# Kolkir/feature-point-cnn

Measured on AMD Instinct MI355X. Metric: frames/sec (VGA 640x480) SuperPoint fwd+NMS+descriptors, higher is better.
Workload: dtype f32

## Files before the change

feature-point-cnn_amd/_lib.py:

```python
import ctypes
import os
import subprocess

import torch

_DIR = os.path.dirname(os.path.abspath(__file__))
LIB_PATH = os.environ.get("FPC_LIB_PATH") or os.path.join(_DIR, "lib", "libfpc.so")
CSRC = os.path.join(_DIR, "csrc")

SYMBOLS = [
    "fpc_abi_version", "fpc_build_flags", "fpc_strerror", "fpc_last_hip_error", "fpc_default_config", "fpc_create",
    "fpc_destroy", "fpc_load_weights", "fpc_packed_size", "fpc_packed_device_ptr",
    "fpc_export_packed", "fpc_import_packed", "fpc_import_packed_device", "fpc_mark_weights_loaded", "fpc_set_stream", "fpc_upload_stream",
    "fpc_get_stream", "fpc_sync", "fpc_forward", "fpc_detect", "fpc_get_points", "fpc_results",
    "fpc_get_counts", "fpc_get_keypoints", "fpc_set_timing", "fpc_get_timings", "fpc_match", "fpc_first_within",
    "fpc_detect_u8", "fpc_u8_staging", "fpc_homography_adaptation", "fpc_detect_u8_resized",
    "fpc_sample_descriptors", "fpc_plan_hash", "fpc_broadcast_weights", "fpc_read_activation",
    "fpc_pack_layout_revision", "fpc_check_guards", "fpc_stream_report", "fpc_output_range",
    "fpc_match_frames", "fpc_first_within_frames",
    "fpc_default_ransac_params", "fpc_ransac_homography", "fpc_homography_frames",
    "fpc_bank_create", "fpc_bank_destroy", "fpc_bank_get", "fpc_bank_store", "fpc_bank_store_rows", "fpc_bank_clear",
    "fpc_match_bank", "fpc_homography_bank", "fpc_bank_create_ex", "fpc_bank_format",
    "fpc_match_frames_guided", "fpc_match_bank_guided",
    "fpc_cell_order", "fpc_match_frames_guided_cells", "fpc_match_bank_guided_cells",
    "fpc_bank_topk_reserve", "fpc_match_bank_topk", "fpc_homography_bank_topk",
    "fpc_ransac_fundamental", "fpc_fundamental_frames", "fpc_fundamental_bank",
    "fpc_match_frames_guided_epipolar", "fpc_match_bank_guided_epipolar",
    "fpc_match_frames_guided_epipolar_cells", "fpc_match_bank_guided_epipolar_cells",
    "fpc_default_pose_params", "fpc_pose_fundamental", "fpc_pose_frames", "fpc_pose_bank",
    "fpc_default_pnp_params", "fpc_pnp_reserve", "fpc_bank_landmarks_reserve", "fpc_bank_store_landmarks",
    "fpc_bank_landmarks_get", "fpc_ransac_pnp", "fpc_pnp_frames", "fpc_pnp_bank",
]

ABI_VERSION = 4
PACK_LAYOUT_REVISION = 4

PLAN_FLAGS = {
    "no_fused_blocks": 1 << 0, "no_winograd": 1 << 1, "no_winograd_detector": 1 << 2, "no_winograd_layer_in1": 1 << 3,
    "no_xcd_order": 1 << 4, "no_fused_stem_pool": 1 << 5, "split_heads": 1 << 6, "nms_in_line": 1 << 7,
    "no_persistent_grid": 1 << 8, "layer1_tile_8x16": 1 << 9, "winograd_gen1": 1 << 10, "no_latency_tiles": 1 << 11,
    "nms_one_workgroup": 1 << 12, "no_fused_softmax": 1 << 13, "winograd_gen2": 1 << 14, "guard_zones": 1 << 15, "detector_gen1": 1 << 16, "heads_in_line": 1 << 17, "w36_one_wave": 1 << 18, "convt_phases": 1 << 19, "stem_round3": 1 << 20, "conv_round1": 1 << 21,
}


class FpcConfig(ctypes.Structure):
    _fields_ = [("device", ctypes.c_int), ("height", ctypes.c_int), ("width", ctypes.c_int),
                ("max_batch", ctypes.c_int), ("cell", ctypes.c_int), ("nms_dist", ctypes.c_int),
                ("conf_thresh", ctypes.c_float), ("border_remove", ctypes.c_int),
                ("descriptor_enabled", ctypes.c_int), ("max_keypoints", ctypes.c_int),
                ("in_channels", ctypes.c_int), ("dtype", ctypes.c_int), ("arch", ctypes.c_int),
                ("num_streams", ctypes.c_int), ("plan_flags", ctypes.c_uint), ("nms_round_launches", ctypes.c_int),
                ("min_sub_batch", ctypes.c_int)]


class FpcTensor(ctypes.Structure):
    _fields_ = [("name", ctypes.c_char_p), ("data", ctypes.c_void_p), ("ndim", ctypes.c_int),
                ("shape", ctypes.c_int64 * 4)]


class FpcDeviceResults(ctypes.Structure):
    _fields_ = [("count", ctypes.c_void_p), ("n_candidates", ctypes.c_void_p), ("xy", ctypes.c_void_p),
                ("conf", ctypes.c_void_p), ("desc", ctypes.c_void_p), ("capacity", ctypes.c_int),
                ("desc_dim", ctypes.c_int)]


class FpcStreamReport(ctypes.Structure):
    _fields_ = [("n_streams", ctypes.c_int), ("slot", ctypes.c_int * 16), ("queue", ctypes.c_int * 16),
                ("probing", ctypes.c_int), ("hw_queues_found", ctypes.c_int), ("process_probe_rounds", ctypes.c_int),
                ("process_probe_launches", ctypes.c_int), ("process_inconclusive_rounds", ctypes.c_int),
                ("process_probe_ms", ctypes.c_float), ("create_probe_rounds", ctypes.c_int),
                ("create_placement_ms", ctypes.c_float), ("process_registered_streams", ctypes.c_int)]


class FpcRansacParams(ctypes.Structure):
    _fields_ = [("iterations", ctypes.c_int), ("reproj_threshold", ctypes.c_float), ("seed", ctypes.c_uint32),
                ("refits", ctypes.c_int), ("min_inliers", ctypes.c_int)]


class FpcPoseParams(ctypes.Structure):
    _fields_ = [("q_fx", ctypes.c_float), ("q_fy", ctypes.c_float), ("q_cx", ctypes.c_float), ("q_cy", ctypes.c_float),
                ("t_fx", ctypes.c_float), ("t_fy", ctypes.c_float), ("t_cx", ctypes.c_float), ("t_cy", ctypes.c_float),
                ("reproj_threshold", ctypes.c_float), ("min_front", ctypes.c_int)]


class FpcPnpParams(ctypes.Structure):
    _fields_ = [("fx", ctypes.c_float), ("fy", ctypes.c_float), ("cx", ctypes.c_float), ("cy", ctypes.c_float),
                ("iterations", ctypes.c_int), ("reproj_threshold", ctypes.c_float), ("seed", ctypes.c_uint32),
                ("refits", ctypes.c_int), ("min_inliers", ctypes.c_int)]


BANK_MAX_SLOTS = 1024
BANK_TOPK_MAX = 16


# ... 73 lines not shown
    l.fpc_first_within_frames.argtypes = [vp, ci, vp, vp, ctypes.c_float, vp]
    rp = ctypes.POINTER(FpcRansacParams)
    l.fpc_default_ransac_params.argtypes = [rp]
    l.fpc_ransac_homography.argtypes = [vp, ci, vp, vp, vp, ci, rp, vp, vp, vp]
    l.fpc_homography_frames.argtypes = [vp, ci, ci, vp, vp, vp, rp, vp, vp, vp]
    l.fpc_bank_create.argtypes = [vp, ci, ci]
    l.fpc_bank_create_ex.argtypes = [vp, ci, ci, ci]
    l.fpc_bank_format.argtypes = [vp, ctypes.POINTER(ci), ctypes.POINTER(vp)]
    l.fpc_bank_destroy.argtypes = [vp]
    l.fpc_bank_get.argtypes = [vp, ctypes.POINTER(FpcBankView)]
    l.fpc_bank_store.argtypes = [vp, ci, ci]
    l.fpc_bank_store_rows.argtypes = [vp, ci, vp, vp, vp]
    l.fpc_bank_clear.argtypes = [vp, ci]
    l.fpc_match_bank.argtypes = [vp, ci, ci, ctypes.c_float, ctypes.c_float, ci, vp, vp, vp, vp]
    l.fpc_homography_bank.argtypes = [vp, ci, vp, vp, rp, vp, vp, vp]
    l.fpc_ransac_fundamental.argtypes = [vp, ci, vp, vp, vp, ci, rp, vp, vp, vp]
    l.fpc_fundamental_frames.argtypes = [vp, ci, ci, vp, vp, vp, rp, vp, vp, vp]
    l.fpc_fundamental_bank.argtypes = [vp, ci, vp, vp, rp, vp, vp, vp]
    pp = ctypes.POINTER(FpcPoseParams)
    l.fpc_default_pose_params.argtypes = [pp]
    l.fpc_pose_fundamental.argtypes = [vp, ci, vp, vp, vp, ci, vp, pp, vp, vp, vp, vp, vp]
    l.fpc_pose_frames.argtypes = [vp, ci, ci, vp, vp, vp, vp, pp, vp, vp, vp, vp, vp]
    l.fpc_pose_bank.argtypes = [vp, ci, vp, vp, vp, pp, vp, vp, vp, vp, vp]
    np_ = ctypes.POINTER(FpcPnpParams)
    l.fpc_default_pnp_params.argtypes = [np_]
    l.fpc_pnp_reserve.argtypes = [vp, ctypes.POINTER(ctypes.c_size_t)]
    l.fpc_bank_landmarks_reserve.argtypes = [vp, ctypes.POINTER(ctypes.c_size_t)]
    l.fpc_bank_store_landmarks.argtypes = [vp, ci, vp, vp]
    l.fpc_bank_landmarks_get.argtypes = [vp, ctypes.POINTER(vp)]
    l.fpc_ransac_pnp.argtypes = [vp, ci, vp, vp, vp, ci, np_, vp, vp, vp, vp]
    l.fpc_pnp_frames.argtypes = [vp, ci, vp, vp, vp, vp, np_, vp, vp, vp, vp]
    l.fpc_pnp_bank.argtypes = [vp, ci, vp, vp, np_, vp, vp, vp, vp]
    l.fpc_match_frames_guided.argtypes = [vp, ci, ci, vp, vp, vp, vp, ctypes.c_float, ci, ctypes.c_float, ctypes.c_float,
                                          vp, vp]
    l.fpc_match_bank_guided.argtypes = [vp, ci, vp, vp, ctypes.c_float, ci, ctypes.c_float, ctypes.c_float, vp, vp]
    l.fpc_cell_order.argtypes = [vp, vp, vp, ci, ci, vp]
    l.fpc_match_frames_guided_cells.argtypes = [vp, ci, ci, vp, vp, vp, vp, ctypes.c_float, ci, ctypes.c_float,
                                                ctypes.c_float, vp, vp, vp]
    l.fpc_match_bank_guided_cells.argtypes = [vp, ci, vp, vp, ctypes.c_float, ci, ctypes.c_float, ctypes.c_float, vp, vp,
                                              vp]
    l.fpc_match_frames_guided_epipolar.argtypes = list(l.fpc_match_frames_guided.argtypes)
    l.fpc_match_bank_guided_epipolar.argtypes = list(l.fpc_match_bank_guided.argtypes)
    l.fpc_match_frames_guided_epipolar_cells.argtypes = list(l.fpc_match_frames_guided_cells.argtypes)
    l.fpc_match_bank_guided_epipolar_cells.argtypes = list(l.fpc_match_bank_guided_cells.argtypes)
    l.fpc_bank_topk_reserve.argtypes = [vp, ci, ctypes.POINTER(ctypes.c_size_t)]
    l.fpc_match_bank_topk.argtypes = [vp, ci, ci, ci, ctypes.c_float, ctypes.c_float, ci, vp, vp, vp, vp, vp]
    l.fpc_homography_bank_topk.argtypes = [vp, ci, ci, vp, vp, rp, vp, vp, vp, vp, vp]
    l.fpc_sample_descriptors.argtypes = [vp, vp, vp, ci, vp]
    l.fpc_read_activation.argtypes = [vp, ctypes.c_char_p, ci, ci, vp, ctypes.POINTER(ci), ctypes.POINTER(ci), ctypes.POINTER(ci)]
    l.fpc_plan_hash.argtypes = [vp]
    l.fpc_plan_hash.restype = ctypes.c_uint64
    l.fpc_broadcast_weights.argtypes = [vp, vp, ci]
    l.fpc_pack_layout_revision.restype = ci
    l.fpc_check_guards.argtypes = [vp, ctypes.POINTER(ctypes.c_longlong)]
    l.fpc_stream_report.argtypes = [vp, ctypes.POINTER(FpcStreamReport)]
    l.fpc_set_timing.argtypes = [vp, ci]
    l.fpc_get_timings.argtypes = [vp, ci, ctypes.POINTER(ctypes.c_char_p), ctypes.POINTER(ctypes.c_char_p),
                                  ctypes.POINTER(ctypes.c_float), ctypes.POINTER(ctypes.c_double),
                                  ctypes.POINTER(ctypes.c_double), ctypes.POINTER(ctypes.c_double)]
    for s in SYMBOLS:
        getattr(l, s)
    if l.fpc_abi_version() != ABI_VERSION:
        raise ImportError("libfpc.so has ABI version %d, this binding is for %d: rebuild (make -C %s)"
                          % (l.fpc_abi_version(), ABI_VERSION, CSRC))
    if l.fpc_pack_layout_revision() != PACK_LAYOUT_REVISION:
        raise ImportError("libfpc.so packs fragment-layout revision %d, this binding expects %d: rebuild (make -C %s)"
                          % (l.fpc_pack_layout_revision(), PACK_LAYOUT_REVISION, CSRC))
    _lib = l
    return l


def check(code, where):
    if code < 0:
        raise FpcError(code, where)
    return code
```

feature-point-cnn_amd/csrc/fpc_api.hip:

```cpp
#include <hip/hip_runtime.h>

#include <dlfcn.h>

#include <algorithm>
#include <cmath>
#include <cstdio>
#include <cstdlib>
#include <cstring>
#include <memory>
#include <mutex>
#include <chrono>
#include <string>
#include <vector>

#include "../../include/fpc.h"
#include "block_mfma.h"
#include "block_bf16.h"
#include "convt_bf16.h"
#include "block_x3.h"
#include "stem_bf16.h"
#include "wblock_mfma.h"
#include "wblock16_mfma.h"
#include "wblock36_mfma.h"
#include "wblock36p_mfma.h"
// ... 70 lines not shown
FPC_KINDS(X)
#undef X

static const KindInfo g_kinds[K_COUNT] = {
#define X(name, TH, TW, S, EXT, KC, WM, WN, MB, NB)                                                    \
  {#name, "conv_mfma_kernel<" #TH ", " #TW ", " #S ", " #EXT ", " #KC ", " #WM ", " #WN ", " #MB ", " #NB ">", TH, TW, S, EXT, KC, WM, WN, MB, NB, ConvCfg<TH, TW, S, EXT, KC, WM, WN, MB, NB>::LDS_BYTES,   \
   WM * WN * 64, (const void*)conv_mfma_kernel<TH, TW, S, EXT, KC, WM, WN, MB, NB>, launch_##name},
    FPC_KINDS(X)
#undef X
};

#define FPC_LEAN_KINDS(X)                          \
  X(T320_2x2_K64_N128, 3, 20, 1, 2, 64, 1, 4, 2, 1) \
  X(T320_1x1_K64_N128, 3, 20, 1, 1, 64, 1, 4, 2, 1)
struct LeanKindInfo {
  Kind kind;
  const char* symbol;
  int lds_bytes;
  const void* fn;
  void (*launch)(const ConvArgs&, dim3, hipStream_t);
};
#define X(name, TH, TW, S, EXT, KC, WM, WN, MB, NB)                                                              \
  static void launch_lean_##name(const ConvArgs& a, dim3 grid, hipStream_t st) {                                 \
    using C2 = Conv2Cfg<TH, TW, S, EXT, KC, WM, WN, MB, NB>;                                                    \
    hipLaunchKernelGGL((conv2_mfma_kernel<TH, TW, S, EXT, KC, WM, WN, MB, NB>), grid, dim3(WM* WN * 64),         \
                       C2::LDS_BYTES, st, a);                                                                    \
  }
FPC_LEAN_KINDS(X)
#undef X
static const LeanKindInfo g_lean_kinds[] = {
#define X(name, TH, TW, S, EXT, KC, WM, WN, MB, NB)                                                                       \
  {K_##name, "conv2_mfma_kernel<" #TH ", " #TW ", " #S ", " #EXT ", " #KC ", " #WM ", " #WN ", " #MB ", " #NB ">",          \
   Conv2Cfg<TH, TW, S, EXT, KC, WM, WN, MB, NB>::LDS_BYTES, (const void*)conv2_mfma_kernel<TH, TW, S, EXT, KC, WM, WN, MB, NB>, \
   launch_lean_##name},
    FPC_LEAN_KINDS(X)
#undef X
};
static const LeanKindInfo* lean_kind(Kind k) {
  for (const LeanKindInfo& l : g_lean_kinds)
    if (l.kind == k) return &l;
  return nullptr;
}

#define FPC_BLOCK_KINDS(X)                                   \
  X(B816_s1_K64_C64, 8, 16, 1, 64, 4, 1, 1, 2, 64)           \
  X(B1616_s1_K32_C64, 16, 16, 1, 32, 4, 1, 2, 2, 64)         \
  X(B620_s2_K32_C128, 6, 20, 2, 32, 2, 2, 2, 2, 128)         \
  X(B620_s1_K64_C128, 6, 20, 1, 64, 2, 2, 2, 2, 128)         \
  X(B620_s1_K64_C72, 6, 20, 1, 64, 4, 1, 1, 3, 72)           \
  X(B620_s1_K72_C72, 6, 20, 1, 72, 4, 1, 1, 3, 72)           \
  X(B320_s2_K32_C256, 3, 20, 2, 32, 1, 4, 2, 2, 256)         \
  X(B310_s2_K32_C256, 3, 10, 2, 32, 1, 4, 1, 2, 256)         \
  X(B320_s2_K32_C128, 3, 20, 2, 32, 1, 4, 2, 1, 128)         \
  X(B320_s1_K64_C256, 3, 20, 1, 64, 1, 4, 2, 2, 256)

enum BKind {
#define X(name, ...) BK_##name,
  FPC_BLOCK_KINDS(X)
#undef X
      BK_COUNT
};

struct BKindInfo {
  const char* name;
  const char* symbol;
  int TH, TW, S, KC, WM, WN, MB, NB, CMIDP;
  int lds_bytes;
  const void* fn;
  void (*launch)(const BlockArgs&, dim3, hipStream_t);
};

#define X(name, TH, TW, S, KC, WM, WN, MB, NB, CMIDP)                                                     \
  static void launchb_##name(const BlockArgs& a, dim3 grid, hipStream_t st) {                             \
    using BC = BlockCfg<TH, TW, S, KC, WM, WN, MB, NB, CMIDP>;                                            \
    hipLaunchKernelGGL((block_mfma_kernel<TH, TW, S, KC, WM, WN, MB, NB, CMIDP>), grid, dim3(WM* WN * 64), \
                       BC::LDS_BYTES, st, a);                                                             \
  }
FPC_BLOCK_KINDS(X)
#undef X

static const BKindInfo g_bkinds[BK_COUNT] = {
#define X(name, TH, TW, S, KC, WM, WN, MB, NB, CMIDP)                                                      \
  {#name, "block_mfma_kernel<" #TH ", " #TW ", " #S ", " #KC ", " #WM ", " #WN ", " #MB ", " #NB ", " #CMIDP ">", \
   TH, TW, S, KC, WM, WN, MB, NB, CMIDP, BlockCfg<TH, TW, S, KC, WM, WN, MB, NB, CMIDP>::LDS_BYTES,         \
   (const void*)block_mfma_kernel<TH, TW, S, KC, WM, WN, MB, NB, CMIDP>, launchb_##name},
    FPC_BLOCK_KINDS(X)
#undef X
};

#define FPC_WBLOCK_KINDS(X)     \
  X(W816_K32_C64, 32, 2, 64)    \
  X(W816_K32_C128, 32, 4, 128)  \
  X(W816_K32_C72, 32, 3, 72)    \
  X(W816_K24_C72, 24, 3, 72)
#define FPC_W16_KINDS(X) \
  X(W16_C64, 4, 8)       \
  X(W16_C128, 8, 8)      \
  X(W16_C128H, 8, 4)
#define FPC_W36_KINDS(X) \
  X(W36_C64_4x4, 1, 4, 4)  \
  X(W36_C64_2x8, 1, 2, 8)  \
  X(W36_C128_4x4, 2, 4, 4) \
  X(W36_C128_2x8, 2, 2, 8)

#define FPC_W36P_KINDS(X) \
  X(W36P_C64_4x4, 4, 4)   \
  X(W36P_C64_2x8, 2, 8)

#define FPC_W36PD_KINDS(X) \
  X(W36PD_C65_4x4, 4, 4)   \
  X(W36PD_C65_2x8, 2, 8)

#define FPC_W36D_KINDS(X) \
  X(W36_C65_4x4, 4, 4)    \
  X(W36_C65_2x8, 2, 8)

enum WKind {
#define X(name, ...) WK_##name,
  FPC_WBLOCK_KINDS(X)
  FPC_W16_KINDS(X)
  FPC_W36_KINDS(X)
  FPC_W36D_KINDS(X)
  FPC_W36P_KINDS(X)
  FPC_W36PD_KINDS(X)
#undef X
      WK_COUNT
};

struct WKindInfo {
  const char* name;
  const char* symbol;
  int gen;
  int KC, NBT, CMID, lds_bytes;
  int NCG;
  int TH;
  int TW;
  int threads;
  const void* fn;
  void (*launch)(const WBlockArgs&, dim3, hipStream_t);
  bool dust = false;
};

#define X(name, KC, NBT, CMID)                                                                            \
  static void launchw_##name(const WBlockArgs& a, dim3 grid, hipStream_t st) {                            \
    constexpr int lds = WBlockCfg<KC, NBT, CMID>::LDS_BYTES;                                              \
    hipLaunchKernelGGL((wblock_mfma_kernel<KC, NBT, CMID>), grid, dim3(512), lds, st, a);                 \
  }
FPC_WBLOCK_KINDS(X)
#undef X
#define X(name, NCG, TH)                                                                                  \
  static void launchw_##name(const WBlockArgs& a, dim3 grid, hipStream_t st) {                            \
    constexpr int lds = W16Cfg<NCG, TH>::LDS_BYTES;                                                       \
    hipLaunchKernelGGL((wblock16_kernel<NCG, TH>), grid, dim3(512), lds, st, a);                          \
  }
FPC_W16_KINDS(X)
#undef X
#define X(name, NB, TYT, TXT)                                                                             \
  static void launchw_##name(const WBlockArgs& a, dim3 grid, hipStream_t st) {                            \
    constexpr int lds = W36Cfg<NB, TYT, TXT>::LDS_BYTES;                                                  \
    hipLaunchKernelGGL((wblock36_kernel<NB, TYT, TXT>), grid, dim3(256), lds, st, a);                     \
  }
FPC_W36_KINDS(X)
#undef X
#define X(name, TYT, TXT)                                                                                  \
  static void launchw_##name(const WBlockArgs& a, dim3 grid, hipStream_t st) {                            \
    constexpr int lds = W36Cfg<1, TYT, TXT, true>::LDS_BYTES;                                             \
    hipLaunchKernelGGL((wblock36_dust_kernel<TYT, TXT>), grid, dim3(256), lds, st, a);                    \
  }
FPC_W36D_KINDS(X)
#undef X
#define X(name, TYT, TXT)                                                                                  \
  static void launchw_##name(const WBlockArgs& a, dim3 grid, hipStream_t st) {                            \
    constexpr int lds = W36PCfg<TYT, TXT>::LDS_BYTES;                                                     \
    hipLaunchKernelGGL((wblock36p_kernel<TYT, TXT>), grid, dim3(512), lds, st, a);                        \
  }
FPC_W36P_KINDS(X)
#undef X
#define X(name, TYT, TXT)                                                                                  \
  static void launchw_##name(const WBlockArgs& a, dim3 grid, hipStream_t st) {                            \
    constexpr int lds = W36PCfg<TYT, TXT, true>::LDS_BYTES;                                               \
    hipLaunchKernelGGL((wblock36p_dust_kernel<TYT, TXT>), grid, dim3(512), lds, st, a);                   \
  }
FPC_W36PD_KINDS(X)
#undef X

static const WKindInfo g_wkinds[WK_COUNT] = {
#define X(name, KC, NBT, CMID)                                                                            \
  {#name, "wblock_mfma_kernel<" #KC ", " #NBT ", " #CMID ">", 1, KC, NBT, CMID,                           \
   WBlockCfg<KC, NBT, CMID>::LDS_BYTES, 0, 8, 16, 512, (const void*)wblock_mfma_kernel<KC, NBT, CMID>, launchw_##name},
    FPC_WBLOCK_KINDS(X)
#undef X
#define X(name, NCG, TH)                                                                                  \
  {#name, "wblock16_kernel<" #NCG ", " #TH ">", 2, 16, NCG / 2, NCG * 16,                                  \
   W16Cfg<NCG, TH>::LDS_BYTES, NCG, TH, 16, 512, (const void*)wblock16_kernel<NCG, TH>, launchw_##name},
    FPC_W16_KINDS(X)
#undef X
#define X(name, NB, TYT, TXT)                                                                             \
  {#name, "wblock36_kernel<" #NB ", " #TYT ", " #TXT ">", 3, 16, 2 * NB, 64 * NB,                          \
   W36Cfg<NB, TYT, TXT>::LDS_BYTES, 4 * NB, 4 * TYT, 4 * TXT, 256, (const void*)wblock36_kernel<NB, TYT, TXT>, launchw_##name},
    FPC_W36_KINDS(X)
#undef X
#define X(name, TYT, TXT)                                                                                 \
  {#name, "wblock36_dust_kernel<" #TYT ", " #TXT ">", 3, 16, 2, 64,                                        \
   W36Cfg<1, TYT, TXT, true>::LDS_BYTES, 4, 4 * TYT, 4 * TXT, 256, (const void*)wblock36_dust_kernel<TYT, TXT>, launchw_##name, true},
    FPC_W36D_KINDS(X)
#undef X
#define X(name, TYT, TXT)                                                                                 \
  {#name, "wblock36p_kernel<" #TYT ", " #TXT ", 3>", 3, 16, 2, 64,                                            \
   W36PCfg<TYT, TXT>::LDS_BYTES, 4, 4 * TYT, 4 * TXT, 512, (const void*)wblock36p_kernel<TYT, TXT>, launchw_##name},
    FPC_W36P_KINDS(X)
#undef X
#define X(name, TYT, TXT)                                                                                 \
  {#name, "wblock36p_dust_kernel<" #TYT ", " #TXT ", 3>", 3, 16, 2, 64,                                    \
   W36PCfg<TYT, TXT, true>::LDS_BYTES, 4, 4 * TYT, 4 * TXT, 512, (const void*)wblock36p_dust_kernel<TYT, TXT>, launchw_##name, true},
    FPC_W36PD_KINDS(X)
#undef X
};

static size_t w1_floats(const WKindInfo& k, int nchunk) {
  if (k.gen == 3) return (size_t)k.NCG * ((size_t)nchunk * 36 + (k.NCG == 8 ? W36Cfg<2, 4, 4>::WPAD : W36Cfg<1, 4, 4>::WPAD)) * 256;
  return (size_t)k.NCG * ((size_t)nchunk * 16 + W16Cfg<8>::WPAD) * 256;
}
static double wkind_mfma_flops(const WKindInfo& k, int tiles, int nchunk, int k8_1x1) {
  const double px = (double)k.TH * k.TW, n = k.NBT * 32.0;
  if (k.gen == 3) return 2.0 * tiles * n * (36.0 * (px / 16) * nchunk * k.KC + px * k8_1x1 * 8.0);
  return 2.0 * tiles * n * (16.0 * (px / 4) * nchunk * k.KC + px * k8_1x1 * 8.0);
}
static bool w36_fits(int , int H, int W, int cs_in, int cs_out) {
  return (unsigned long long)H * W * (unsigned long long)std::max(cs_in, cs_out) * sizeof(float) < (unsigned long long)W36_MARKER;
}
static int w36_frames_per_launch(int H, int W, int cs_in, int cs_out) {
  const unsigned long long fb = (unsigned long long)H * W * (unsigned long long)std::max(cs_in, cs_out) * sizeof(float);
  return (int)std::max<unsigned long long>(1, ((unsigned long long)W36_MARKER - 1) / fb);
}
static int w36_conv_part(int cout, int tiles, int cus) {
  if (cout < 128) return 64;
  if (cout == 128) return 128;
  const double t2 = std::ceil((double)tiles * (cout / 128) / cus) * 1.0, t1 = std::ceil((double)tiles * (cout / 64) / cus) * 0.53;
  return t1 < t2 ? 64 : 128;
}
static WKind w36_kind(int cout, int H, int W, bool paired = false) {
  const int t44 = ((H + 15) / 16) * ((W + 15) / 16), t28 = ((H + 7) / 8) * ((W + 31) / 32);
  if (cout == 65 && paired) return t28 < t44 ? WK_W36PD_C65_2x8 : WK_W36PD_C65_4x4;
  if (cout == 65) return t28 < t44 ? WK_W36_C65_2x8 : WK_W36_C65_4x4;
  if (cout == 64 && paired) return t28 < t44 ? WK_W36P_C64_2x8 : WK_W36P_C64_4x4;
  if (cout == 64) return t28 < t44 ? WK_W36_C64_2x8 : WK_W36_C64_4x4;
  return t28 < t44 ? WK_W36_C128_2x8 : WK_W36_C128_4x4;
}

#define FPC_BF16_KINDS(X)                                                                   \
  X(F816_s1_K64_C64, block_bf16_one_kernel, BlockBfCfg, 1, 8, 32, 1, 3, 64, 2, 2, 4, 1, 64) \
  X(F816_s1_K64_C128, block_bf16_kernel, BlockBfCfg, 1, 8, 16, 1, 3, 64, 1, 4, 4, 1, 128)   \
  X(F816_s1_K80_C80, block_bf16_one_kernel, BlockBfCfg, 1, 8, 16, 1, 3, 80, 4, 1, 1, 3, 80) \
  X(F816_s1_K128_C128, block_bf16_one_kernel, BlockBfCfg, 1, 8, 16, 1, 3, 128, 1, 4, 4, 1, 128) \
  X(F816_s1_K128_C80w, block_bf16_one_kernel, BlockBfCfg, 1, 8, 16, 1, 3, 128, 1, 4, 4, 1, 80) \
  X(F620_s2_K64_C128, block_bf16_one_kernel, BlockBfCfg, 1, 6, 20, 2, 3, 64, 2, 2, 2, 2, 128) \
  X(F320_s2_K128_C256, block_bf16_one_kernel, BlockBfCfg, 1, 3, 20, 2, 3, 128, 1, 4, 2, 2, 256) \
  X(F416_s1_K128_C256, block_bf16_two_kernel, BlockBfCfg, 1, 4, 16, 1, 3, 128, 1, 4, 2, 2, 256) \
  X(F816_ct_K64_C128, block_bf16_kernel, BlockBfCfg, 1, 8, 16, 1, 2, 64, 1, 4, 4, 1, 128)   \
  X(F816_ctf_K64_C128, convt_bf16_kernel, ConvTBfCfg, 1, 8, 16, 1, 2, 64, 2, 2, 2, 1, 128)  \
  X(S816_s1_K64_C64, block_x3_kernel, BlockX3Cfg, 3, 8, 16, 1, 3, 64, 2, 2, 2, 1, 64)       \
  X(S620_s2_K16_C128, block_x3_kernel, BlockX3Cfg, 3, 6, 20, 2, 3, 16, 2, 2, 2, 2, 128)     \
  X(S620_s1_K64_C128, block_x3_kernel, BlockX3Cfg, 3, 6, 20, 1, 3, 64, 2, 2, 2, 2, 128)     \
  X(S620_s1_K64_C80, block_x3_kernel, BlockX3Cfg, 3, 6, 20, 1, 3, 64, 4, 1, 1, 3, 80)       \
  X(S620_s1_K16_C80, block_x3_kernel, BlockX3Cfg, 3, 6, 20, 1, 3, 16, 4, 1, 1, 3, 80)       \
  X(S320_s2_K16_C256, block_x3_kernel, BlockX3Cfg, 3, 3, 20, 2, 3, 16, 1, 4, 2, 2, 256)     \
  X(S320_s1_K64_C256, block_x3_kernel, BlockX3Cfg, 3, 3, 20, 1, 3, 64, 1, 4, 2, 2, 256)     \
  X(S620_ct_K64_C128, block_x3_kernel, BlockX3Cfg, 3, 6, 20, 1, 2, 64, 2, 2, 2, 2, 128)     \
  X(S620_1x1_K64_C80, block_x3_kernel, BlockX3Cfg, 3, 6, 20, 1, 1, 64, 4, 1, 1, 3, 80)      \
  X(S320_1x1_K64_C256, block_x3_kernel, BlockX3Cfg, 3, 3, 20, 1, 1, 64, 1, 4, 2, 2, 256)     \
  X(H816_s1_K64_C64, block_h2_kernel, BlockH2Cfg, 2, 8, 16, 1, 3, 64, 2, 2, 2, 1, 64)     \
  X(H620_s2_K16_C128, block_h2_kernel, BlockH2Cfg, 2, 6, 20, 2, 3, 16, 2, 2, 2, 2, 128)     \
  X(H620_s1_K64_C128, block_h2_kernel, BlockH2Cfg, 2, 6, 20, 1, 3, 64, 2, 2, 2, 2, 128)     \
  X(H620_s1_K64_C80, block_h2_kernel, BlockH2Cfg, 2, 6, 20, 1, 3, 64, 4, 1, 1, 3, 80)     \
  X(H620_s1_K16_C80, block_h2_kernel, BlockH2Cfg, 2, 6, 20, 1, 3, 16, 4, 1, 1, 3, 80)     \
  X(H320_s2_K16_C256, block_h2_kernel, BlockH2Cfg, 2, 3, 20, 2, 3, 16, 1, 4, 2, 2, 256)     \
  X(H320_s1_K64_C256, block_h2_kernel, BlockH2Cfg, 2, 3, 20, 1, 3, 64, 1, 4, 2, 2, 256)     \
  X(H620_ct_K64_C128, block_h2_kernel, BlockH2Cfg, 2, 6, 20, 1, 2, 64, 2, 2, 2, 2, 128)     \
  X(H620_1x1_K64_C80, block_h2_kernel, BlockH2Cfg, 2, 6, 20, 1, 1, 64, 4, 1, 1, 3, 80)     \
  X(H320_1x1_K64_C256, block_h2_kernel, BlockH2Cfg, 2, 3, 20, 1, 1, 64, 1, 4, 2, 2, 256)

enum FKind {
#define X(name, ...) FK_##name,
  FPC_BF16_KINDS(X)
#undef X
      FK_COUNT
};

struct FKindInfo {
  const char* name;
  const char* symbol;
  int planes, TH, TW, S, EXT, KC, WM, WN, MB, NB, CMIDP;
  int lds_bytes;
  const void* fn;
  void (*launch)(const BlockBfArgs&, dim3, hipStream_t);
};

#define X(name, KERN, CFG, PL, TH, TW, S, EXT, KC, WM, WN, MB, NB, CMIDP)                                  \
  static void launchf_##name(const BlockBfArgs& a, dim3 grid, hipStream_t st) {                            \
    constexpr int lds = CFG<TH, TW, S, EXT, KC, WM, WN, MB, NB, CMIDP>::LDS_BYTES;                         \
    hipLaunchKernelGGL((KERN<TH, TW, S, EXT, KC, WM, WN, MB, NB, CMIDP>), grid, dim3(WM* WN * 64), lds, st, a); \
  }
FPC_BF16_KINDS(X)
#undef X

static const FKindInfo g_fkinds[FK_COUNT] = {
#define X(name, KERN, CFG, PL, TH, TW, S, EXT, KC, WM, WN, MB, NB, CMIDP)                                   \
  {#name, #KERN "<" #TH ", " #TW ", " #S ", " #EXT ", " #KC ", " #WM ", " #WN ", " #MB ", " #NB ", " #CMIDP ">", \
   PL, TH, TW, S, EXT, KC, WM, WN, MB, NB, CMIDP, CFG<TH, TW, S, EXT, KC, WM, WN, MB, NB, CMIDP>::LDS_BYTES,   \
   (const void*)KERN<TH, TW, S, EXT, KC, WM, WN, MB, NB, CMIDP>, launchf_##name},
    FPC_BF16_KINDS(X)
#undef X
};

enum OpType { OP_STEM, OP_POOL, OP_CONV, OP_BLOCK, OP_WBLOCK, OP_BF16, OP_SOFTMAX, OP_NMS, OP_DESC,
              OP_VCONV0, OP_POOL2, OP_L2NORM };

struct Op {
  OpType type;
  std::string name;
  Kind kind = K_COUNT;
  ConvArgs args{};
  BKind bkind = BK_COUNT;
  BlockArgs bargs{};
  WKind wkind = WK_COUNT;
  WBlockArgs wargs{};
  FKind fkind = FK_COUNT;
  BlockBfArgs fargs{};
  int phase = -1;
  int when = 0;
  bool shadow = false;
  bool wconv = false;
  int n0 = 0;
  bool plain_conv = false;
  bool lean = false;
  int ksize = 0;
  const float* pin = nullptr;
  float* pout = nullptr;
  int pH = 0, pW = 0, pC = 0;
  std::string prefix;
  int cin = 0, cout = 0;
  int grid_y = 1, grid_z = 1;
  double flops_per_frame = 0;
  double mfma_flops_per_frame = 0;
  bool fused_softmax_capable = false;
  double bytes_per_frame = 0;
  bool descriptor_branch = false;
};

struct Timing {
  hipEvent_t start, stop;
  int op;
  int frames;
};

}

using namespace fpc;

struct fpc_ctx {
  fpc_config cfg{};
  int H = 0, W = 0, B = 0, Hc = 0, Wc = 0;
  bool vgg = false;
  int D = 128;
  std::vector<float*> vbuf;
  size_t vconv0_off = 0;
  bool bf16 = false;
  bool split = false;
  bool split_f16 = false;
  int lgcs = 72;
  int cin = 3;
  int cap = 0, sort_cap = 0;
  hipStream_t stream = nullptr;
  bool own_stream = false;
  hipStream_t upload = nullptr;
  bool queue_probe = true;
  int probe_rounds = 0;
  double placement_ms = 0.0;
  std::vector<std::pair<hipStream_t, int>> caller_stream_memo;
  std::vector<hipStream_t> aux;
  std::vector<hipEvent_t> ev_join;
  std::vector<hipStream_t> side;
  std::vector<hipEvent_t> ev_enc, ev_det;
  bool nms_aside = true;
  bool split_heads = false;
  hipEvent_t ev_fork = nullptr;
  int min_sub = 8;
  int num_cus = 256;
  int fkind_blocks_per_cu[64] = {};
  int persist_min_tiles = 1;
  bool xcd_order = true;
  int nms_passes = 2;
  bool fuse_softmax = true;
  bool convt_fused = true;
  bool logits_valid = false;
  bool nms_one_workgroup = false;
  int nms_g = 0;
  bool fuse_stem_pool = true;
  bool conv_lean = true;
  bool stem_lean = true;
  bool stem2 = false;
  bool layer1_t816 = false;
#ifdef FPC_DIAG
  unsigned long long* diag_stamps = nullptr;
  int diag_n = 0;
#endif
  bool winograd_in1 = true;
  bool winograd_det = true;
  int w36_cus = 0;
  bool w36_paired = true;
  bool winograd_det_gen3 = true;
  bool winograd = true;
  bool latency_tiles = true;
  int winograd_gen = 3;
  bool fuse_blocks = true;
  bool weights_loaded = false;
  bool plan_error = false;

  char* slab = nullptr;
  size_t slab_bytes = 0;
  bool guard_zones = false;
  std::vector<std::pair<size_t, size_t>> guards;
  float *stem_out, *x0, *h4, *x1, *x2, *h8, *x3, *cat, *dh, *dproj, *d0, *lg;
  float *h16, *y16a, *y16b, *lo_h, *lo0, *desc_map, *desc_in_nhwc;
  float* prob;
  uint32_t *nmsmap, *cand;
  int32_t *ncand, *count, *xy, *status;
  float* rowmax = nullptr;
  uint32_t* range = nullptr;
  float *conf, *desc_out;
  unsigned long long* sort_scratch;
  int32_t* nms_aux = nullptr;
  unsigned long long *rowbest, *colbest;
  float* mf_norms = nullptr;
  unsigned long long *mf_top2 = nullptr, *mf_colbest = nullptr;
  float4* hf_pairs = nullptr;
  int32_t *hf_row = nullptr, *hf_np = nullptr;
  unsigned long long* hf_best = nullptr;
  int32_t *mgc_perm_q = nullptr, *mgc_perm_t = nullptr;
  int4* mgc_box = nullptr;
  char* bank_slab = nullptr;
  size_t bank_bytes = 0;
  BankArgs bank{};
  int bank_format = FPC_BANK_F32;
  BankBf16Args bank16{};
  std::vector<std::pair<size_t, size_t>> bank_guards;
  char* topk_slab = nullptr;
  BankTopkArgs topk{};
  float4* topk_pairs = nullptr;
  int32_t *topk_row = nullptr, *topk_np = nullptr;
  unsigned long long* topk_best = nullptr;
  std::vector<std::pair<size_t, size_t>> topk_guards;
  char* pnp_slab = nullptr;
  float4* pnp_rec = nullptr;
  int32_t* pnp_np = nullptr;
  unsigned long long* pnp_best = nullptr;
  std::vector<std::pair<size_t, size_t>> pnp_guards;
  char* lm_slab = nullptr;
  float4* lm_xyzw = nullptr;
  std::vector<std::pair<size_t, size_t>> lm_guards;
  int pts_n = 0;
  bool pts_desc = false;
// ... 213 lines not shown
  float* out;
  int cso, cout, cout_pad;
  bool proj, desc_branch;
};

static void add_block(fpc_ctx* c, const BlockSpec& s, size_t* blob_off) {
  const BKindInfo& k = g_bkinds[s.kind];
  Op op;
  op.type = OP_BLOCK;
  op.name = s.prefix + (s.proj ? " [conv1+bn1+relu+conv2+bn2+proj+relu]" : " [conv1+bn1+relu+conv2+bn2+identity+relu]");
  op.prefix = s.prefix;
  op.bkind = s.kind;
  op.cin = s.cin;
  op.cout = s.cout;
  op.descriptor_branch = s.desc_branch;
  BlockArgs& a = op.bargs;
  const int nbt = k.WN * k.NB, K8 = k.KC / 8;
  a.x = s.x;
  a.csx = s.csx;
  a.x_bytes = (unsigned)std::min<size_t>((size_t)c->B * s.H * s.W * s.csx * 4, 0xffffff00u);
  a.nchunk = s.cin_pad / k.KC;
  a.H = s.H;
  a.W = s.W;
  const int HWp = (k.TW - 1) * k.S + 3, ROW4 = k.KC / 4 + 1;
  for (int ky = 0; ky < 3; ++ky)
    for (int kx = 0; kx < 3; ++kx) a.tapoff4[ky * 3 + kx] = (ky * HWp + kx) * ROW4;
  a.k8_h = k.CMIDP / 8;
  a.k8_x = s.proj ? s.cin_pad / 8 : 0;
  if (a.k8_x % 8) { fprintf(stderr, "fpc: fused block %s: projection over %d channels is not a multiple of 64\n", s.prefix.c_str(), s.cin_pad); abort(); }
  a.out = s.out;
  a.cso = s.cso;
  a.Ho = s.H / k.S;
  a.Wo = s.W / k.S;
  a.tiles_x = (a.Wo + k.TW - 1) / k.TW;
  a.tiles_y = (a.Ho + k.TH - 1) / k.TH;
  a.nstore = s.cout_pad;
  fpc_ctx::ConvW cw;
  cw.w_off[0] = *blob_off;
  *blob_off += ((size_t)a.nchunk * 9 * K8 + 2) * nbt * 64 * 4;
  cw.b_off = *blob_off;
  *blob_off += (size_t)nbt * 32;
  cw.w_off[1] = *blob_off;
  *blob_off += ((size_t)(a.k8_h + a.k8_x) + 2) * nbt * 64 * 4;
  cw.b2_off = *blob_off;
  *blob_off += (size_t)nbt * 32;
  op.flops_per_frame = 2.0 * a.Ho * a.Wo * s.cout * ((double)s.cin * 9 + s.cout + (s.proj ? s.cin : 0));
  op.mfma_flops_per_frame = 2.0 * a.tiles_x * a.tiles_y * (k.WM * k.MB * 32.0) * (nbt * 32.0) *
                            ((double)a.nchunk * k.KC * 9 + (a.k8_h + a.k8_x) * 8.0);
  op.bytes_per_frame = 4.0 * ((double)s.cin * s.H * s.W + (double)s.cout * a.Ho * a.Wo);
  c->ops.push_back(op);
  c->convw.push_back(cw);
}

static void retile_last(fpc_ctx* c, BKind small) {
  if (!c->latency_tiles || c->ops.empty() || c->ops.back().type != OP_BLOCK) return;
  const BKindInfo &k0 = g_bkinds[c->ops.back().bkind], &k = g_bkinds[small];
  if (k.KC != k0.KC || k.WN * k.NB != k0.WN * k0.NB || k.S != k0.S || k.CMIDP != k0.CMIDP) { c->plan_error = true; return; }
  Op& o = c->ops.back();
  o.bkind = small;
  BlockArgs& a = o.bargs;
  const int HWp = (k.TW - 1) * k.S + 3, ROW4 = k.KC / 4 + 1;
  for (int ky = 0; ky < 3; ++ky)
    for (int kx = 0; kx < 3; ++kx) a.tapoff4[ky * 3 + kx] = (ky * HWp + kx) * ROW4;
  a.tiles_x = (a.Wo + k.TW - 1) / k.TW;
  a.tiles_y = (a.Ho + k.TH - 1) / k.TH;
  o.mfma_flops_per_frame = 2.0 * a.tiles_x * a.tiles_y * (k.WM * k.MB * 32.0) * (k.WN * k.NB * 32.0) *
                           ((double)a.nchunk * k.KC * 9 + (a.k8_h + a.k8_x) * 8.0);
}

static void retile_last(fpc_ctx* c, Kind small) {
  if (!c->latency_tiles || c->ops.empty() || c->ops.back().type != OP_CONV) return;
  const KindInfo &k0 = g_kinds[c->ops.back().kind], &k = g_kinds[small];
  if (k.KC != k0.KC || k.WN * k.NB != k0.WN * k0.NB || k.S != k0.S || k.EXT != k0.EXT) { c->plan_error = true; return; }
  Op& o = c->ops.back();
  o.kind = small;
  ConvArgs& a = o.args;
  const int HWp = (k.TW - 1) * k.S + k.EXT, HWp0 = (k0.TW - 1) * k0.S + k0.EXT, ROW4 = k.KC / 4 + 1;
  for (int z = 0; z < o.grid_z; ++z)
    for (int t = 0; t < a.sub[z].ntaps; ++t) {
      const int lin = a.sub[z].tapoff4[t] / ROW4, dy = lin / HWp0, dx = lin - dy * HWp0;
      a.sub[z].tapoff4[t] = (dy * HWp + dx) * ROW4;
    }
  a.tiles_x = (a.Wo + k.TW - 1) / k.TW;
  a.tiles_y = (a.Ho + k.TH - 1) / k.TH;
  o.lean = conv_is_lean(c, o);
}

static void add_wblock(fpc_ctx* c, const BlockSpec& s, WKind wk, size_t* blob_off, bool small_only = false) {
  const WKindInfo& k = g_wkinds[wk];
  Op op;
  op.type = OP_WBLOCK;
  op.name = s.prefix + (s.proj ? " [winograd conv1+bn1+relu+conv2+bn2+proj+relu]" : " [winograd conv1+bn1+relu+conv2+bn2+identity+relu]");
  op.prefix = s.prefix;
  op.wkind = wk;
  op.cin = s.cin;
  op.cout = s.cout;
  op.descriptor_branch = s.desc_branch;
  WBlockArgs& a = op.wargs;
  const int K8 = k.KC / 8;
  a.x = s.x;
  a.csx = s.csx;
  a.nchunk = s.cin_pad / k.KC;
  a.dust = nullptr;
  a.dust_in = 0;
  if (k.dust) {
    if (s.cout != 65 || !(s.cin == 65 ? !s.proj : (s.cin == s.cin_pad && s.cin_pad % 64 == 0 && s.cin_pad <= 256))) { c->plan_error = true; return; }
    a.dust_in = s.cin == 65;
    a.nchunk = a.dust_in ? 4 : s.cin_pad / 16;
  } else if (s.cin_pad % k.KC) { c->plan_error = true; return; }
  a.H = s.H;
  a.W = s.W;
  a.k8_h = k.CMID / 8;
  a.k8_x = s.proj ? s.cin_pad / 8 : 0;
  if (a.k8_x % 4) { fprintf(stderr, "fpc: winograd block %s: projection over %d channels is not a multiple of 32\n", s.prefix.c_str(), s.cin_pad); abort(); }
  a.out = s.out;
  a.cso = s.cso;
  a.tiles_x = (s.W + k.TW - 1) / k.TW;
  a.tiles_y = (s.H + k.TH - 1) / k.TH;
  fpc_ctx::ConvW cw;
  cw.w_off[0] = *blob_off;
// ... 17 lines not shown
  op.flops_per_frame = 2.0 * s.H * s.W * s.cout * ((double)s.cin * 9 + s.cout + (s.proj ? s.cin : 0));
  op.mfma_flops_per_frame = wkind_mfma_flops(k, a.tiles_x * a.tiles_y, a.nchunk, a.k8_h + a.k8_x);
  if (k.dust && a.dust_in) op.mfma_flops_per_frame += 2.0 * a.tiles_x * a.tiles_y * 64.0 * 36 * 16 * 4;
  op.bytes_per_frame = 4.0 * ((double)s.cin * s.H * s.W + (double)s.cout * s.H * s.W);
  if (k.dust) {
    op.when = c->latency_tiles ? 2 : 0;
    c->ops.push_back(op);
    c->convw.push_back(cw);
    if (c->latency_tiles) add_wblock(c, s, s.cin == 65 ? WK_W816_K24_C72 : WK_W816_K32_C72, blob_off, true);
    return;
  }
  if (k.gen == 3 && c->latency_tiles) {
    op.when = 2;
    c->ops.push_back(op);
    c->convw.push_back(cw);
    add_wblock(c, s, s.cout == 64 ? WK_W16_C64 : WK_W16_C128, blob_off, true);
    return;
  }
  if (small_only && wk == WK_W16_C128) {
    const WKindInfo& kh = g_wkinds[WK_W16_C128H];
    op.when = 1;
    op.wkind = WK_W16_C128H;
    op.wargs.tiles_y = (s.H + kh.TH - 1) / kh.TH;
    op.mfma_flops_per_frame = wkind_mfma_flops(kh, op.wargs.tiles_x * op.wargs.tiles_y, a.nchunk, a.k8_h + a.k8_x);
    c->ops.push_back(op);
    c->convw.push_back(cw);
    return;
  }
  if (small_only) op.when = 1;
  c->ops.push_back(op);
  c->convw.push_back(cw);
  if (wk == WK_W16_C128 && c->latency_tiles) {
    const WKindInfo& kh = g_wkinds[WK_W16_C128H];
    c->ops.back().when = 2;
    Op oh = c->ops.back();
    oh.when = 1;
    oh.wkind = WK_W16_C128H;
    oh.wargs.tiles_y = (s.H + kh.TH - 1) / kh.TH;
    oh.mfma_flops_per_frame = wkind_mfma_flops(kh, oh.wargs.tiles_x * oh.wargs.tiles_y, a.nchunk, a.k8_h + a.k8_x);
    c->ops.push_back(oh);
    c->convw.push_back(cw);
  }
}

static void add_wconv(fpc_ctx* c, const std::string& prefix, bool bn, WKind wk, const float* x, int csx, int cin, int H,
                      int W, float* out, int cso, int cout, int n0, bool desc_branch, size_t* blob_off) {
  const WKindInfo& k = g_wkinds[wk];
  Op op;
  op.type = OP_WBLOCK;
  op.name = prefix + (bn ? ".conv1+bn1+relu [winograd" : " [winograd conv+bias+relu") +
            (cout > k.CMID ? ", channels " + std::to_string(n0) + ".." + std::to_string(n0 + k.CMID - 1) : std::string()) + "]";
  op.prefix = prefix;
  op.wkind = wk;
  op.wconv = true;
  op.plain_conv = !bn;
  op.n0 = n0;
  op.cin = cin;
  op.cout = cout;
  op.descriptor_branch = desc_branch;
  WBlockArgs& a = op.wargs;
  const int K8 = k.KC / 8;
  a.x = x;
  a.csx = csx;
  a.nchunk = cin / k.KC;
  a.H = H;
  a.W = W;
  a.k8_h = a.k8_x = 0;
  a.conv_only = 1;
  a.out = out + n0;
  a.cso = cso;
  a.tiles_x = (W + k.TW - 1) / k.TW;
  a.tiles_y = (H + k.TH - 1) / k.TH;
  fpc_ctx::ConvW cw;
  cw.w_off[0] = *blob_off;
  if (k.gen >= 2) {
    if (a.nchunk < 4 || (a.nchunk & 1)) { c->plan_error = true; return; }
    *blob_off += w1_floats(k, a.nchunk);
  } else {
    *blob_off += ((size_t)a.nchunk * 16 * K8 + 16 * K8 + 2) * k.NBT * 64 * 4;
  }
  cw.b_off = *blob_off;
  *blob_off += (size_t)k.NBT * 32;
  op.flops_per_frame = 2.0 * H * W * (double)k.CMID * cin * 9;
  op.mfma_flops_per_frame = wkind_mfma_flops(k, a.tiles_x * a.tiles_y, a.nchunk, 0);
  op.bytes_per_frame = 4.0 * ((double)cin * H * W + (double)std::min(k.CMID, cout - n0) * H * W);
  const int part = n0 / k.CMID;
  if (k.gen >= 2 && part > 0 && n0 % k.CMID == 0 && cout % k.CMID == 0 && (int)c->ops.size() >= part) {
    Op& first = c->ops[c->ops.size() - part];
    fpc_ctx::ConvW& cf = c->convw[c->convw.size() - part];
    if (first.wconv && first.prefix == prefix && first.n0 == 0 && first.wkind == wk && first.grid_y == part) {
      const int ys = (int)((cw.w_off[0] - cf.w_off[0]) / part);
      if (part == 1) first.wargs.ysplit_floats = ys;
      else if (first.wargs.ysplit_floats != ys) { c->plan_error = true; return; }
      first.grid_y = part + 1;
      first.flops_per_frame += op.flops_per_frame;
      first.mfma_flops_per_frame += op.mfma_flops_per_frame;
      first.bytes_per_frame = 4.0 * ((double)cin * H * W + (double)std::min(cout, (part + 1) * k.CMID) * H * W);
      const std::string parts = std::to_string(part + 1) + " parts of " + std::to_string(k.CMID) + " channels";
      first.name = prefix + (bn ? ".conv1+bn1+relu [winograd, " : " [winograd conv+bias+relu, ") + parts + "]";
      op.shadow = true;
    }
  }
  c->ops.push_back(op);
  c->convw.push_back(cw);
}

// ... 602 lines not shown
      WKind wk = WK_COUNT;
      if (c->winograd && stride == 1) {
        const int gen = c->winograd_gen == 3 && (!w36_fits(c->B, Hx, Wx, csx, csy) || (proj && cinp % 64 != 0)) ? 2 : c->winograd_gen;
        if (cinp % 32 == 0 && cout == 64) wk = gen == 3 ? w36_kind(64, Hx, Wx, c->w36_paired) : gen == 2 ? WK_W16_C64 : WK_W816_K32_C64;
        else if (cinp % 32 == 0 && cout == 128) wk = gen == 3 ? w36_kind(128, Hx, Wx) : gen == 2 ? WK_W16_C128 : WK_W816_K32_C128;
        else if (c->winograd_det && cout == 65 && c->winograd_det_gen3 && c->winograd_gen == 3 && w36_fits(c->B, Hx, Wx, csx, csy) &&
                 (cin == 65 ? !proj : (cin == cinp && cinp % 64 == 0 && cinp <= 256)))
          wk = w36_kind(65, Hx, Wx, c->w36_paired);
        else if (c->winograd_det && cinp % 32 == 0 && coutp == 72) wk = WK_W816_K32_C72;
        else if (c->winograd_det && cinp == 72 && coutp == 72) wk = WK_W816_K24_C72;
      }
      if (wk != WK_COUNT)
        add_wblock(c, bs, wk, &bo);
      else
        add_block(c, bs, &bo);
      return;
    }
    const int Ho = Hx / stride, Wo = Wx / stride;
    ConvSpec s{};
    s.name = p + ".conv1+bn1+relu";
    s.kind = k3; s.ksize = 3; s.stride = stride;
    s.in0 = x; s.cs0 = csx; s.cin0 = cin; s.cin0_pad = cinp; s.H0 = Hx; s.W0 = Wx;
    s.out = h; s.cso = csh; s.cout = cout; s.nstore = coutp; s.Ho = Ho; s.Wo = Wo; s.relu = 1;
    s.desc_branch = desc;
    add_conv(c, s, &bo);
    ConvSpec t{};
    t.name = p + (proj ? ".conv2+bn2+proj+relu" : ".conv2+bn2+identity+relu");
    t.kind = k1; t.ksize = 1; t.stride = 1;
    t.in0 = h; t.cs0 = csh; t.cin0 = cout; t.cin0_pad = coutp; t.H0 = Ho; t.W0 = Wo;
    if (proj) {
      t.in1 = x; t.cs1 = csx; t.cin1 = cin; t.cin1_pad = cinp; t.s1 = stride; t.H1 = Hx; t.W1 = Wx;
    } else {
      t.res = x; t.csr = csx;
    }
    t.out = y; t.cso = csy; t.cout = cout; t.nstore = coutp; t.Ho = Ho; t.Wo = Wo; t.relu = 1;
    t.desc_branch = desc;
    add_conv(c, t, &bo);
  };
  float* feat = c->cat + 128;
  if (c->bf16 || c->split) {
    if (c->bf16) build_bf16_ops(c, &bo);
    else build_x3_ops(c, &bo);
    goto postproc;
  }
  {
  const BKind l1kind = c->layer1_t816 ? BK_B816_s1_K64_C64 : BK_B1616_s1_K32_C64;
  block("encoder.layer1.0", K_T816_3x3_K64_N64, K_T816_1x1_K64_N64, 1, c->x0, 64, 64, 64, H4, W4, c->h4, 64, 64, 64,
        c->x1, 64, true, false, l1kind);
  block("encoder.layer1.1", K_T816_3x3_K64_N64, K_T816_1x1_K64_N64, 1, c->x1, 64, 64, 64, H4, W4, c->h4, 64, 64, 64,
        c->x2, 64, false, false, l1kind);
  block("encoder.layer2.0", K_T620_3x3s2_K32_N128, K_T620_1x1_K64_N128, 2, c->x2, 64, 64, 64, H4, W4, c->h8, 128,
        128, 128, c->x3, 128, true, false, BK_B620_s2_K32_C128);
  if (c->fuse_blocks) retile_last(c, BK_B320_s2_K32_C128);
  block("encoder.layer2.1", K_T620_3x3_K64_N128, K_T620_1x1_K64_N128, 1, c->x3, 128, 128, 128, Hc, Wc, c->h8, 128,
        128, 128, feat, 256, false, false, BK_B620_s1_K64_C128);
  if (c->fuse_blocks) {
    const BlockSpec bs{"detector.layer.0", BK_B620_s1_K64_C72, feat, 256, 128, 128, Hc, Wc, c->d0, 72, 65, 72, true, false};
    if (c->winograd && c->winograd_det)
      add_wblock(c, bs, c->winograd_det_gen3 && c->winograd_gen == 3 && w36_fits(c->B, Hc, Wc, 256, 72) ? w36_kind(65, Hc, Wc, c->w36_paired) : WK_W816_K32_C72, &bo);
    else add_block(c, bs, &bo);
  } else {
    ConvSpec s{};
    s.name = "detector.layer.0.conv1+bn1+relu";
    s.kind = K_T620_3x3_K64_N96; s.ksize = 3; s.stride = 1;
    s.in0 = feat; s.cs0 = 256; s.cin0 = 128; s.cin0_pad = 128; s.H0 = Hc; s.W0 = Wc;
    s.out = c->dh; s.cso = 72; s.cout = 65; s.nstore = 72; s.Ho = Hc; s.Wo = Wc; s.relu = 1;
    add_conv(c, s, &bo);
    ConvSpec p{};
    p.name = "detector.layer.0.identity_downsample";
    p.kind = K_T620_1x1_K64_N96; p.ksize = 1; p.stride = 1;
    p.in0 = feat; p.cs0 = 256; p.cin0 = 128; p.cin0_pad = 128; p.H0 = Hc; p.W0 = Wc;
    p.out = c->dproj; p.cso = 72; p.cout = 65; p.nstore = 72; p.Ho = Hc; p.Wo = Wc; p.relu = 0;
    add_conv(c, p, &bo);
    ConvSpec t{};
    t.name = "detector.layer.0.conv2+bn2+shortcut+relu";
    t.kind = K_T620_1x1_K72_N96; t.ksize = 1; t.stride = 1;
    t.in0 = c->dh; t.cs0 = 72; t.cin0 = 65; t.cin0_pad = 72; t.H0 = Hc; t.W0 = Wc;
    t.res = c->dproj; t.csr = 72;
    t.out = c->d0; t.cso = 72; t.cout = 65; t.nstore = 72; t.Ho = Hc; t.Wo = Wc; t.relu = 1;
    add_conv(c, t, &bo);
  }
  block("detector.layer.1", K_T620_3x3_K72_N96, K_T620_1x1_K72_N96, 1, c->d0, 72, 65, 72, Hc, Wc, c->dh, 72, 65, 72,
        c->lg, 72, false, false, BK_B620_s1_K72_C72);
  {
    Op op;
    op.type = OP_SOFTMAX;
    op.name = "exp-softmax+depth_to_space+threshold";
    c->ops.push_back(op);
    c->convw.push_back({});
  }
  if (de) {
    block("descriptor.layer_in.0", K_T620_3x3s2_K32_N128, K_T620_1x1_K64_N128, 2, feat, 256, 128, 128, Hc, Wc, c->h16,
          256, 256, 256, c->y16a, 256, true, true, BK_B320_s2_K32_C256);
    if (c->fuse_blocks) retile_last(c, BK_B310_s2_K32_C256);
    if (c->fuse_blocks && c->winograd && c->winograd_in1) {
      const std::string p = "descriptor.layer_in.1";
      const bool g3 = c->winograd_gen == 3 && w36_fits(c->B, H16, W16, 256, 256);
      const int in1_parts = g3 ? 4 : 2;
      for (int n0 = 0; n0 < 256; n0 += 256 / in1_parts)
        add_wconv(c, p, true, g3 ? w36_kind(64, H16, W16, c->w36_paired) : c->winograd_gen >= 2 ? WK_W16_C128 : WK_W816_K32_C128, c->y16a, 256, 256, H16, W16, c->h16, 256, 256, n0, true, &bo);
      const size_t in1_ops = in1_parts + 1;
      ConvSpec t{};
      t.name = p + ".conv2+bn2+identity+relu";
      t.kind = K_T620_1x1_K64_N128; t.ksize = 1; t.stride = 1;
      t.in0 = c->h16; t.cs0 = 256; t.cin0 = 256; t.cin0_pad = 256; t.H0 = H16; t.W0 = W16;
      t.res = c->y16a; t.csr = 256;
      t.out = c->y16b; t.cso = 256; t.cout = 256; t.nstore = 256; t.Ho = H16; t.Wo = W16; t.relu = 1;
      t.desc_branch = true;
      add_conv(c, t, &bo);
      retile_last(c, K_T320_1x1_K64_N128);
      if (g_wkinds[c->ops[c->ops.size() - in1_ops].wkind].gen == 2 && c->latency_tiles) {
        const size_t ia = c->ops.size() - in1_ops;
        c->ops[ia].when = 2;
        Op oh = c->ops[ia];
        oh.when = 1;
        oh.wkind = WK_W16_C128H;
        oh.wargs.tiles_y = (H16 + 3) / 4;
        oh.mfma_flops_per_frame = 2 * 2.0 * oh.wargs.tiles_x * oh.wargs.tiles_y * 128.0 * (16.0 * 16 * 256);
        const fpc_ctx::ConvW cwa = c->convw[ia];
        c->ops.insert(c->ops.begin() + ia + 1, oh);
        c->convw.insert(c->convw.begin() + ia + 1, cwa);
      } else if (g_wkinds[c->ops[c->ops.size() - in1_ops].wkind].gen == 3 && c->latency_tiles) {
        for (size_t k = c->ops.size() - in1_ops; k < c->ops.size(); ++k) c->ops[k].when = 2;
        const size_t ib = c->ops.size();
        for (int n0 = 0; n0 < 256; n0 += 128)
          add_wconv(c, p, true, WK_W16_C128, c->y16a, 256, 256, H16, W16, c->h16, 256, 256, n0, true, &bo);
        add_conv(c, t, &bo);
        retile_last(c, K_T320_1x1_K64_N128);
        Op& oh = c->ops[ib];
        oh.wkind = WK_W16_C128H;
        oh.wargs.tiles_y = (H16 + 3) / 4;
        oh.mfma_flops_per_frame = 2 * 2.0 * oh.wargs.tiles_x * oh.wargs.tiles_y * 128.0 * (16.0 * 16 * 256);
        for (size_t k = ib; k < c->ops.size(); ++k) c->ops[k].when = 1;
      } else if (c->latency_tiles || c->winograd_gen == 1) {
      for (size_t k = c->ops.size() - in1_ops; k < c->ops.size(); ++k) c->ops[k].when = 2;
      block("descriptor.layer_in.1", K_T620_3x3_K64_N128, K_T620_1x1_K64_N128, 1, c->y16a, 256, 256, 256, H16, W16,
            c->h16, 256, 256, 256, c->y16b, 256, false, true, BK_B320_s1_K64_C256);
      c->ops.back().when = 1;
      }
    } else
    block("descriptor.layer_in.1", K_T620_3x3_K64_N128, K_T620_1x1_K64_N128, 1, c->y16a, 256, 256, 256, H16, W16,
          c->h16, 256, 256, 256, c->y16b, 256, false, true, BK_B320_s1_K64_C256);
    ConvSpec u{};
    u.name = "descriptor.up_sample+bn+relu";
    u.kind = K_T620_2x2_K64_N128; u.ksize = 2; u.stride = 1;
    u.in0 = c->y16b; u.cs0 = 256; u.cin0 = 256; u.cin0_pad = 256; u.H0 = H16; u.W0 = W16;
    u.out = c->cat; u.cso = 256; u.cout = 128; u.nstore = 128; u.Ho = Hc; u.Wo = Wc; u.relu = 1;
    u.desc_branch = true;
    add_conv(c, u, &bo);
    retile_last(c, K_T320_2x2_K64_N128);
    block("descriptor.layer_out.0", K_T620_3x3_K64_N128, K_T620_1x1_K64_N128, 1, c->cat, 256, 256, 256, Hc, Wc,
          c->lo_h, 128, 128, 128, c->lo0, 128, true, true, BK_B620_s1_K64_C128);
    block("descriptor.layer_out.1", K_T620_3x3_K64_N128, K_T620_1x1_K64_N128, 1, c->lo0, 128, 128, 128, Hc, Wc,
// ... 18 lines not shown
    if (op.type == OP_SOFTMAX) op.bytes_per_frame = 4.0 * (65.0 * Hc * Wc + 2.0 * H * W);
  c->blob_floats = bo;
  HIPCHECK(hipMalloc((void**)&c->blob, c->blob_floats * sizeof(float)));
  HIPCHECK(hipMemset(c->blob, 0, c->blob_floats * sizeof(float)));
  for (size_t i = 0; i < c->ops.size(); ++i) {
    Op& op = c->ops[i];
    if (op.type == OP_WBLOCK) {
      op.wargs.w1 = reinterpret_cast<const float4*>(c->blob + c->convw[i].w_off[0]);
      op.wargs.b1 = c->blob + c->convw[i].b_off;
      op.wargs.w2 = reinterpret_cast<const float4*>(c->blob + c->convw[i].w_off[1]);
      op.wargs.b2 = c->blob + c->convw[i].b2_off;
      op.wargs.dust = g_wkinds[op.wkind].dust ? c->blob + c->convw[i].w_off[2] : nullptr;
    }
    if (op.type == OP_BF16) {
      op.fargs.w1 = reinterpret_cast<const uint4*>(c->blob + c->convw[i].w_off[0]);
      op.fargs.b1 = c->blob + c->convw[i].b_off;
      op.fargs.w2 = reinterpret_cast<const uint4*>(c->blob + c->convw[i].w_off[1]);
      op.fargs.b2 = c->blob + c->convw[i].b2_off;
    }
    if (op.type == OP_BLOCK) {
      op.bargs.w1 = reinterpret_cast<const float4*>(c->blob + c->convw[i].w_off[0]);
      op.bargs.b1 = c->blob + c->convw[i].b_off;
      op.bargs.w2 = reinterpret_cast<const float4*>(c->blob + c->convw[i].w_off[1]);
      op.bargs.b2 = c->blob + c->convw[i].b2_off;
    }
    if (op.type != OP_CONV) continue;
    for (int z = 0; z < op.grid_z; ++z)
      op.args.sub[z].wfrag = reinterpret_cast<const float4*>(c->blob + c->convw[i].w_off[z]);
    op.args.bias = c->blob + c->convw[i].b_off;
  }
  c->stem.wfrag = reinterpret_cast<const float4*>(c->blob + c->stem_w_off);
  c->stem.bias = c->blob + c->stem_b_off;
  c->stem.out = c->stem_out;
  c->stem.H = H; c->stem.W = W; c->stem.Ho = H2; c->stem.Wo = W2;
  c->stem.tiles_x = (W2 + STEM_T - 1) / STEM_T;
  c->stem.tiles_y = (H2 + STEM_T - 1) / STEM_T;
  c->stem2 = c->stem_lean && !c->bf16 && !c->split && !c->vgg && (c->fuse_stem_pool || c->cin == 1) && H2 % 2 == 0 && W2 % STEM_T == 0;
  return FPC_OK;
}

static uint64_t plan_hash(const fpc_ctx* c) {
  uint64_t h = 1469598103934665603ull;
  auto mix = [&](uint64_t v) {
    for (int i = 0; i < 8; ++i) {
      h ^= (v >> (8 * i)) & 0xff;
      h *= 1099511628211ull;
    }
  };
  mix(FPC_ABI_VERSION); mix(FPC_PACK_LAYOUT_REVISION); mix((uint64_t)c->cfg.dtype); mix((uint64_t)c->cfg.arch); mix((uint64_t)c->cin);
  mix((uint64_t)(c->cfg.descriptor_enabled != 0)); mix(c->blob_floats); mix(c->stem_w_off); mix(c->stem_b_off);
  mix(c->vconv0_off);
  for (size_t i = 0; i < c->ops.size(); ++i) {
    const Op& op = c->ops[i];
    mix((uint64_t)op.type); mix((uint64_t)op.kind); mix((uint64_t)op.bkind); mix((uint64_t)op.wkind); mix((uint64_t)op.fkind);
    mix((uint64_t)(op.phase + 1)); mix((uint64_t)op.n0);
    for (char ch : op.prefix) mix((uint64_t)(unsigned char)ch);
    const fpc_ctx::ConvW& cw = c->convw[i];
    for (int z = 0; z < 4; ++z) mix(cw.w_off[z]);
    mix(cw.b_off); mix(cw.b2_off);
  }
  return h;
}

static void fill_blob_header(const fpc_ctx* c, uint32_t* h) {
  memset(h, 0, BLOB_HEADER_FLOATS * sizeof(uint32_t));
  const uint64_t ph = plan_hash(c);
  h[0] = BLOB_MAGIC; h[1] = FPC_ABI_VERSION; h[2] = (uint32_t)c->cfg.dtype; h[3] = (uint32_t)c->cfg.arch;
  h[4] = (uint32_t)ph; h[5] = (uint32_t)(ph >> 32);
  h[6] = (uint32_t)c->blob_floats; h[7] = (uint32_t)((uint64_t)c->blob_floats >> 32);
  h[8] = 1;
  h[9] = FPC_PACK_LAYOUT_REVISION;
}

static bool check_blob_header(const fpc_ctx* c, const uint32_t* h, std::string* why) {
  uint32_t want[BLOB_HEADER_FLOATS];
  fill_blob_header(c, want);
  static const char* what[10] = {"magic", "ABI version", "dtype", "arch", "launch plan", "launch plan", "size", "size", "weights-present flag",
                                 "fragment-layout revision"};
  for (int i = 0; i < 10; ++i)
    if (h[i] != want[i]) {
      *why = std::string("packed weights do not match this context: ") + what[i] + " differs (the blob was packed by another "
             "build, dtype, arch or plan, or holds no weights)";
      return false;
    }
  return true;
}

static std::vector<double> winograd_filters(const float* w1, int n0, int nn, int ci, const std::vector<double>& scale, int P) {
  static const double G2[4][3] = {{1, 0, 0}, {0.5, 0.5, 0.5}, {0.5, -0.5, 0.5}, {0, 0, 1}};
  static const double G4[6][3] = {{1.0 / 4, 0, 0},          {-1.0 / 6, -1.0 / 6, -1.0 / 6}, {-1.0 / 6, 1.0 / 6, -1.0 / 6},
                                  {1.0 / 24, 1.0 / 12, 1.0 / 6}, {1.0 / 24, -1.0 / 12, 1.0 / 6}, {0, 0, 1}};
  const int R = P == 36 ? 6 : 4;
  const double(*G)[3] = P == 36 ? G4 : G2;
  std::vector<double> U((size_t)nn * ci * P);
  for (int n = 0; n < nn; ++n)
    for (int cc = 0; cc < ci; ++cc) {
      const float* g = w1 + ((size_t)(n0 + n) * ci + cc) * 9;
      double t[6][3];
      for (int i = 0; i < R; ++i)
        for (int j = 0; j < 3; ++j) t[i][j] = G[i][0] * g[0 * 3 + j] + G[i][1] * g[1 * 3 + j] + G[i][2] * g[2 * 3 + j];
      for (int i = 0; i < R; ++i)
        for (int j = 0; j < R; ++j)
          U[((size_t)n * ci + cc) * P + i * R + j] = (t[i][0] * G[j][0] + t[i][1] * G[j][1] + t[i][2] * G[j][2]) * scale[n0 + n];
    }
  return U;
}

// ... 421 lines not shown
      std::vector<PackSource> srcs;
      srcs.push_back({co, cin0p, 1, [&, co](int n, int c_, int) { return (double)w[(size_t)n * co + c_]; }, &f.s});
      for (int n = 0; n < co; ++n) bias[n] = f.t[n];
      const float* wp = nullptr;
      int cip = 0;
      if (a.in1) {
        auto ip = m.find(p + ".identity_downsample.0.weight");
        if (ip == m.end() || ip->second.shape.size() != 4 || (int)ip->second.shape[0] != co || !ip->second.data ||
            (int)ip->second.shape[1] > cin1p) {
          if (missing->empty()) *missing = p + ".identity_downsample.0.weight";
          return FPC_E_MISSING_KEY;
        }
        wp = ip->second.data;
        cip = (int)ip->second.shape[1];
        if (!fold_bn(m, p + ".identity_downsample.1", co, &fp, missing)) return FPC_E_MISSING_KEY;
        srcs.push_back({cip, cin1p, 1, [&, cip](int n, int c_, int) { return (double)wp[(size_t)n * cip + c_]; }, &fp.s});
        for (int n = 0; n < co; ++n) bias[n] += fp.t[n];
      }
      std::vector<float> frag = pack_conv(srcs, co, a.nbt, k.KC);
      memcpy(blob.data() + cw.w_off[0], frag.data(), frag.size() * sizeof(float));
    } else {
      *missing = "internal: unknown op " + nm;
      return FPC_E_INVALID;
    }
    for (int n = 0; n < a.nbt * 32; ++n) blob[cw.b_off + n] = (float)bias[n];
  }
  return FPC_OK;
}

static hipEvent_t next_event(fpc_ctx* c) {
  if (c->events_used == c->event_pool.size()) {
    hipEvent_t e;
    hipEventCreate(&e);
    c->event_pool.push_back(e);
  }
  return c->event_pool[c->events_used++];
}

struct Sub {
  int f0, n;
  bool small = false;
  bool fuse_softmax = false;
  hipStream_t st;
  hipStream_t side = nullptr;
  hipEvent_t ev_enc = nullptr, ev_det = nullptr;
};

struct LaunchTimer {
  fpc_ctx* c;
  int op;
  hipStream_t st;
  int frames;
  hipEvent_t s{}, e{};
  LaunchTimer(fpc_ctx* c_, int op_, hipStream_t st_, int frames_) : c(c_), op(op_), st(st_), frames(frames_) {
    if (c->timing) {
      s = next_event(c);
      e = next_event(c);
      hipEventRecord(s, st);
    }
  }
  ~LaunchTimer() {
    if (c->timing) {
      hipEventRecord(e, st);
      c->timings.push_back({s, e, op, frames});
    }
  }
};

static int op_index(const fpc_ctx* c, OpType t) {
  for (size_t i = 0; i < c->ops.size(); ++i)
    if (c->ops[i].type == t) return (int)i;
  return -1;
}

static void run_network(fpc_ctx* c, const float* frames, const Sub& sb0, int which, hipStream_t st) {
  Sub sb = sb0;
  sb.st = st;
  const int H = c->H, W = c->W, n = sb.n, f0 = sb.f0;
  for (size_t i = 0; i < c->ops.size(); ++i) {
    const Op& op = c->ops[i];
    const int br = op.descriptor_branch ? 2 : (op.name.compare(0, 8, "detector") == 0 ? 1 : 0);
    if (br != which) continue;
    if (op.shadow) continue;
    if (op.when == 1 && !sb.small) continue;
    if (op.when == 2 && sb.small) continue;
    switch (op.type) {
      case OP_STEM: {
        if (c->fuse_stem_pool || c->cin == 1 || c->bf16) {
          float* x0 = c->bf16 ? reinterpret_cast<float*>(reinterpret_cast<unsigned short*>(c->x0) + (size_t)f0 * (H / 4) * (W / 4) * 64)
                              : c->x0 + (size_t)f0 * (H / 4) * (W / 4) * 64;
          if (!c->bf16) stem_border_clear_kernel<<<(n * (H / 4) + 7) / 8, 256, 0, sb.st>>>(reinterpret_cast<float4*>(x0), H / 4, W / 4, n * (H / 4));
          LaunchTimer t(c, (int)i, sb.st, n);
          StemPoolArgs a{};
          a.in = frames + (size_t)f0 * c->cin * H * W;
          a.wfrag = c->stem.wfrag;
          a.bias = c->stem.bias;
          a.out = x0;
          a.H = H; a.W = W; a.Ho = H / 2; a.Wo = W / 2; a.Hp = H / 4; a.Wp = W / 4;
          a.tiles_x = c->stem.tiles_x; a.tiles_y = c->stem.tiles_y;
          a.range = c->range + (size_t)f0 * FPC_RANGE_WORDS;
          if (c->split || c->bf16) {
            StemX3Args x{};
            x.in = a.in; x.wfrag = reinterpret_cast<const uint4*>(a.wfrag); x.bias = a.bias; x.out = a.out;
            x.H = H; x.W = W; x.Ho = a.Ho; x.Wo = a.Wo; x.Hp = a.Hp; x.Wp = a.Wp; x.tiles_x = a.tiles_x; x.tiles_y = a.tiles_y;
            x.range_flag = c->split_f16 ? c->status + 1 : nullptr;
#ifdef FPC_DIAG
            x.stamps = nullptr;
            if (const char* e = getenv("FPC_STAMP_OP"))
              if (op.name.find(e) != std::string::npos) {
                if (!c->diag_stamps) hipHostMalloc((void**)&c->diag_stamps, (size_t)65536 * 8 * sizeof(unsigned long long));
                memset(c->diag_stamps, 0, (size_t)65536 * 8 * sizeof(unsigned long long));
                x.stamps = c->diag_stamps;
                c->diag_n = a.tiles_x * a.tiles_y * n;
              }
#endif
            const dim3 grid(a.tiles_x * a.tiles_y * n);
            if (c->split_f16) {
// ... 12 lines not shown
              else hipLaunchKernelGGL((stem_pool_x3_kernel<3, 3>), grid, dim3(256), 0, sb.st, x);
            }
          } else if (c->stem2) {
            if (c->cin == 1) hipLaunchKernelGGL(stem_pool2_kernel<1>, dim3(a.tiles_x * a.tiles_y * n), dim3(256), 0, sb.st, a);
            else hipLaunchKernelGGL(stem_pool2_kernel<3>, dim3(a.tiles_x * a.tiles_y * n), dim3(256), 0, sb.st, a);
          } else if (c->cin == 1)
            hipLaunchKernelGGL(stem_pool_kernel<1>, dim3(a.tiles_x * a.tiles_y * n), dim3(256), 0, sb.st, a);
          else
            hipLaunchKernelGGL(stem_pool_kernel<3>, dim3(a.tiles_x * a.tiles_y * n), dim3(256), 0, sb.st, a);
          break;
        }
        LaunchTimer t(c, (int)i, sb.st, n);
        StemArgs a = c->stem;
        a.in = frames + (size_t)f0 * 3 * H * W;
        a.out = c->stem_out + (size_t)f0 * (H / 2) * (W / 2) * 64;
        hipLaunchKernelGGL(stem_kernel, dim3(a.tiles_x * a.tiles_y * n), dim3(256), 0, sb.st, a);
        break;
      }
      case OP_POOL: {
        if (c->fuse_stem_pool || c->cin == 1 || c->bf16) break;
        LaunchTimer t(c, (int)i, sb.st, n);
        const size_t total = (size_t)n * (H / 4) * (W / 4) * 16;
        hipLaunchKernelGGL(maxpool_kernel, dim3((unsigned)((total + 255) / 256)), dim3(256), 0, sb.st,
                           reinterpret_cast<const float4*>(c->stem_out + (size_t)f0 * (H / 2) * (W / 2) * 64),
                           reinterpret_cast<float4*>(c->x0 + (size_t)f0 * (H / 4) * (W / 4) * 64), n, H / 2, W / 2, H / 4,
                           W / 4);
        break;
      }
      case OP_WBLOCK: {
        LaunchTimer t(c, (int)i, sb.st, n);
        WBlockArgs a = op.wargs;
        a.frame0 = f0;
#ifdef FPC_DIAG
        a.stamps = nullptr;
        if (const char* e = getenv("FPC_STAMP_OP"))
          if (op.name.find(e) != std::string::npos) {
            if (!c->diag_stamps) hipHostMalloc((void**)&c->diag_stamps, (size_t)65536 * 8 * sizeof(unsigned long long));
            memset(c->diag_stamps, 0, (size_t)65536 * 8 * sizeof(unsigned long long));
            a.stamps = c->diag_stamps;
            c->diag_n = a.tiles_x * a.tiles_y * n;
          }
#endif
        a.total = a.tiles_x * a.tiles_y * n;
        a.xcd_order = c->xcd_order ? 1 : 0;
        {
          const unsigned long long xb = (unsigned long long)(f0 + n) * a.H * a.W * a.csx * sizeof(float);
          a.x_bytes = xb > 0xfffffff0ull ? 0xfffffff0u : (unsigned)xb;
        }
        int grid = (c->persist_min_tiles > 0 && a.total >= c->persist_min_tiles * c->num_cus) ? c->num_cus : a.total;
        if (g_wkinds[op.wkind].gen == 3) {
          const int fpl = w36_frames_per_launch(a.H, a.W, a.csx, a.cso);
          const float* x0 = a.x;
          float* o0 = a.out;
          for (int g0 = 0; g0 < n; g0 += fpl) {
            const int gn = std::min(fpl, n - g0);
            a.frame0 = 0;
            a.x = x0 + (size_t)(f0 + g0) * a.H * a.W * a.csx;
            a.out = o0 + (size_t)(f0 + g0) * a.H * a.W * a.cso;
            a.total = a.tiles_x * a.tiles_y * gn;
            a.x_bytes = (unsigned)((unsigned long long)gn * a.H * a.W * a.csx * sizeof(float));
            const int cus_cap = c->w36_cus > 0 ? std::min(c->num_cus, c->w36_cus) : c->num_cus;
            const int cus8 = std::max(1, cus_cap / 8 / std::max(1, op.grid_y)), per_xcd = (a.total + 7) / 8;
            const int rounds = (per_xcd + cus8 - 1) / cus8;
            const int grid3 = 8 * std::min(cus8, (per_xcd + rounds - 1) / rounds);
            g_wkinds[op.wkind].launch(a, dim3(std::min(a.total, grid3), op.grid_y), sb.st);
          }
          break;
        }
        g_wkinds[op.wkind].launch(a, dim3(std::min(a.total, grid), op.grid_y), sb.st);
        break;
      }
      case OP_BLOCK: {
        LaunchTimer t(c, (int)i, sb.st, n);
        BlockArgs a = op.bargs;
        a.frame0 = f0;
#ifdef FPC_DIAG
        a.stamps = nullptr;
        if (const char* e = getenv("FPC_STAMP_OP"))
          if (op.name.find(e) != std::string::npos) {
            if (!c->diag_stamps) hipHostMalloc((void**)&c->diag_stamps, (size_t)65536 * 8 * sizeof(unsigned long long));
            memset(c->diag_stamps, 0, (size_t)65536 * 8 * sizeof(unsigned long long));
            a.stamps = c->diag_stamps;
            c->diag_n = a.tiles_x * a.tiles_y * n;
          }
#endif
        g_bkinds[op.bkind].launch(a, dim3(a.tiles_x * a.tiles_y * n), sb.st);
        break;
      }
      case OP_BF16: {
        LaunchTimer t(c, (int)i, sb.st, n);
        BlockBfArgs a = op.fargs;
        a.frame0 = f0;
        a.range_flag = c->split_f16 ? c->status + 1 : nullptr;
#ifdef FPC_DIAG
        a.stamps = nullptr;
        if (const char* e = getenv("FPC_STAMP_OP"))
          if (op.name.find(e) != std::string::npos) {
            if (!c->diag_stamps) hipHostMalloc((void**)&c->diag_stamps, (size_t)65536 * 8 * sizeof(unsigned long long));
            memset(c->diag_stamps, 0, (size_t)65536 * 8 * sizeof(unsigned long long));
            a.stamps = c->diag_stamps;
            c->diag_n = a.tiles_x * a.tiles_y * n;
          }
#endif
        if (g_fkinds[op.fkind].planes == 1) {
          a.total_tiles = a.tiles_x * a.tiles_y * n;
          if (sb.fuse_softmax && op.fused_softmax_capable) {
            const size_t HW = (size_t)c->H * c->W;
            hipMemsetAsync(c->ncand + f0, 0, sizeof(int32_t) * n, sb.st);
            a.softmax = 1;
            a.thresh = c->cfg.conf_thresh;
            a.nmsmap = c->nmsmap + f0 * HW;
            a.cand = c->cand + f0 * HW;
            a.ncand = c->ncand + f0;
          }
          const int g = std::min((a.total_tiles + 7) / 8 * 8, std::max(8, c->fkind_blocks_per_cu[op.fkind] * c->num_cus / op.grid_y / 8 * 8));
          g_fkinds[op.fkind].launch(a, dim3(g, op.grid_y), sb.st);
        } else {
          g_fkinds[op.fkind].launch(a, dim3(a.tiles_x * a.tiles_y * n), sb.st);
        }
// ... 297 lines not shown
      cfg->width > 3328)
    return FPC_E_INVALID;
  int ndev = 0;
  if (hipGetDeviceCount(&ndev) != hipSuccess || ndev <= 0 || cfg->device < 0 || cfg->device >= ndev) {
    g_hip_err = "hipGetDeviceCount: no device";
    return FPC_E_NO_DEVICE;
  }
  HIPCHECK(hipSetDevice(cfg->device));
  std::unique_ptr<fpc_ctx> c(new fpc_ctx());
  {
    hipDeviceProp_t prop;
    HIPCHECK(hipGetDeviceProperties(&prop, cfg->device));
    c->num_cus = std::max(1, prop.multiProcessorCount);
  }
  c->cfg = *cfg;
  c->H = cfg->height;
  c->W = cfg->width;
  c->B = cfg->max_batch;
  c->Hc = c->H / 8;
  c->Wc = c->W / 8;
  c->cin = cfg->in_channels == 1 ? 1 : 3;
  c->vgg = cfg->arch == FPC_ARCH_VGG;
  c->D = c->vgg ? 256 : 128;
  c->bf16 = cfg->dtype == FPC_BF16;
  c->split = cfg->dtype == FPC_F32_SPLIT || cfg->dtype == FPC_F32_SPLIT_F16;
  c->split_f16 = cfg->dtype == FPC_F32_SPLIT_F16;
  c->lgcs = (c->bf16 || c->split) ? 80 : 72;
  const int r1 = cfg->nms_dist + 1;
  const int worst = ((c->H + r1 - 1) / r1) * ((c->W + r1 - 1) / r1);
  c->cap = cfg->max_keypoints > 0 ? cfg->max_keypoints : worst;
  c->sort_cap = 1;
  while (c->sort_cap < worst) c->sort_cap <<= 1;
  {
    const int prc = prepare_kernels(c.get(), cfg);
    if (prc != FPC_OK) return prc;
  }
  const bool qprobe = qmap::probe_mode() != 0;
  c->queue_probe = qprobe;
  const auto create_t0 = std::chrono::steady_clock::now();
  std::unique_lock<std::mutex> queue_lock(qmap::state().mu);
  const int probe_rounds0 = qmap::state().dev[cfg->device].rounds;
  c->stream = qmap::acquire(cfg->device, c.get(), SLOT_MAIN, true, qprobe, true);
  if (!c->stream) { qmap::release_owner(c.get()); g_hip_err = "hipStreamCreateWithFlags"; return FPC_E_HIP; }
  c->own_stream = true;
  {
    int nsub = cfg->num_streams > 0 ? std::min(8, cfg->num_streams) : (c->split ? 3 : 2);
    const unsigned pf = cfg->plan_flags;
    c->fuse_blocks = !(pf & FPC_PLAN_NO_FUSED_BLOCKS);
    c->guard_zones = (pf & FPC_PLAN_GUARD_ZONES) != 0;
    if (const char* e = getenv("FPC_GUARD_ZONES")) c->guard_zones = atoi(e) != 0;
    c->winograd_det_gen3 = !(pf & FPC_PLAN_DETECTOR_GEN1);
    c->w36_paired = !(pf & FPC_PLAN_W36_ONE_WAVE);
    if (const char* e = getenv("FPC_W36_PAIRED")) c->w36_paired = atoi(e) != 0;
    if (const char* e = getenv("FPC_W36_CUS")) c->w36_cus = std::max(0, atoi(e));
    if (const char* e = getenv("FPC_WINOGRAD_DET_GEN")) c->winograd_det_gen3 = atoi(e) >= 3;
    c->winograd = !(pf & FPC_PLAN_NO_WINOGRAD);
    c->winograd_det = !(pf & FPC_PLAN_NO_WINOGRAD_DETECTOR);
    c->winograd_in1 = !(pf & FPC_PLAN_NO_WINOGRAD_LAYER_IN1);
    c->xcd_order = !(pf & FPC_PLAN_NO_XCD_ORDER);
    c->fuse_stem_pool = !(pf & FPC_PLAN_NO_FUSED_STEM_POOL);
    c->stem_lean = !(pf & FPC_PLAN_STEM_ROUND3);
    c->conv_lean = !(pf & FPC_PLAN_CONV_ROUND1);
    if (const char* e = getenv("FPC_CONV_LEAN")) c->conv_lean = atoi(e) != 0;
    if (const char* e = getenv("FPC_STEM_LEAN")) c->stem_lean = atoi(e) != 0;
    c->split_heads = (pf & FPC_PLAN_SPLIT_HEADS) != 0;
    if (pf & FPC_PLAN_NO_PERSISTENT_GRID) c->persist_min_tiles = 0;
    c->layer1_t816 = (pf & FPC_PLAN_LAYER1_TILE_8x16) != 0;
    c->winograd_gen = (pf & FPC_PLAN_WINOGRAD_GEN1) ? 1 : (pf & FPC_PLAN_WINOGRAD_GEN2) ? 2 : 3;
    if (const char* e = getenv("FPC_WINOGRAD_GEN")) c->winograd_gen = std::min(3, std::max(1, atoi(e)));
    c->latency_tiles = !(pf & FPC_PLAN_NO_LATENCY_TILES);
    if (const char* e = getenv("FPC_LATENCY_TILES")) c->latency_tiles = atoi(e) != 0;
    c->fuse_softmax = !(pf & FPC_PLAN_NO_FUSED_SOFTMAX);
    c->convt_fused = !(pf & FPC_PLAN_CONVT_PHASES);
    if (const char* e = getenv("FPC_CONVT_FUSED")) c->convt_fused = atoi(e) != 0;
    if (const char* e = getenv("FPC_FUSE_SOFTMAX")) c->fuse_softmax = atoi(e) != 0;
    c->nms_one_workgroup = (pf & FPC_PLAN_NMS_ONE_WORKGROUP) != 0;
    if (const char* e = getenv("FPC_NMS_CHUNKED")) c->nms_one_workgroup = atoi(e) == 0;
    if (cfg->min_sub_batch > 0) c->min_sub = cfg->min_sub_batch;
    if (cfg->nms_round_launches > 0) c->nms_passes = std::min(64, cfg->nms_round_launches);
    else if (cfg->nms_round_launches < 0) c->nms_passes = 0;
    if (const char* e = getenv("FPC_STREAMS")) nsub = std::max(1, std::min(8, atoi(e)));
    if (!(pf & FPC_PLAN_HEADS_IN_LINE) && nsub >= 2 && !c->vgg && !c->bf16 && !c->split) c->split_heads = true;
    if (const char* e = getenv("FPC_FUSE")) c->fuse_blocks = atoi(e) != 0;
    if (const char* e = getenv("FPC_WINOGRAD")) c->winograd = atoi(e) != 0;
    if (const char* e = getenv("FPC_XCD_ORDER")) c->xcd_order = atoi(e) != 0;
    if (const char* e = getenv("FPC_MIN_SUB")) c->min_sub = std::max(1, atoi(e));
    if (const char* e = getenv("FPC_PERSIST_MIN")) c->persist_min_tiles = atoi(e);
    if (const char* e = getenv("FPC_WINOGRAD_DET")) c->winograd_det = atoi(e) != 0;
    if (const char* e = getenv("FPC_WINOGRAD_IN1")) c->winograd_in1 = atoi(e) != 0;
    if (const char* e = getenv("FPC_FUSE_STEM")) c->fuse_stem_pool = atoi(e) != 0;
    if (const char* e = getenv("FPC_NMS_PASSES")) c->nms_passes = std::max(0, std::min(64, atoi(e)));
    if (const char* e = getenv("FPC_NMS_G")) c->nms_g = std::max(0, std::min(64, atoi(e)));
    if (getenv("FPC_L1_T816")) c->layer1_t816 = true;
    auto fail = [&](const char* what) {
      g_hip_err = what;
      queue_lock.unlock();
      fpc_destroy(c.release());
      return FPC_E_HIP;
    };
    if (hipEventCreateWithFlags(&c->ev_fork, hipEventDisableTiming) != hipSuccess) return fail("hipEventCreateWithFlags");
    for (int i = 1; i < nsub; ++i) {
      hipStream_t st = qmap::acquire(cfg->device, c.get(), SLOT_AUX + (i - 1), true, qprobe, true);
      hipEvent_t ev;
      if (!st) return fail("hipStreamCreateWithFlags");
      c->aux.push_back(st);
      if (hipEventCreateWithFlags(&ev, hipEventDisableTiming) != hipSuccess) return fail("hipEventCreateWithFlags");
// ... 105 lines not shown
  if (cap < c->blob_floats * sizeof(float)) return FPC_E_CAPACITY;
  HIPCHECK(hipSetDevice(c->cfg.device));
  HIPCHECK(hipMemcpy(dst, c->blob, c->blob_floats * sizeof(float), hipMemcpyDeviceToHost));
  return FPC_OK;
}

int fpc_import_packed(fpc_ctx* c, const void* src, size_t n) {
  if (!c || !src) return FPC_E_INVALID;
  if (n != c->blob_floats * sizeof(float)) {
    g_hip_err = "packed weights: " + std::to_string(n) + " bytes, this context's plan packs " + std::to_string(c->blob_floats * sizeof(float));
    return FPC_E_INVALID;
  }
  if (!check_blob_header(c, static_cast<const uint32_t*>(src), &g_hip_err)) return FPC_E_INVALID;
  HIPCHECK(hipSetDevice(c->cfg.device));
  HIPCHECK(hipMemcpy(c->blob, src, n, hipMemcpyHostToDevice));
  c->weights_loaded = true;
  return FPC_OK;
}

int fpc_import_packed_device(fpc_ctx* c, const void* src_dev, size_t n) {
  if (!c || !src_dev) return FPC_E_INVALID;
  if (n != c->blob_floats * sizeof(float)) {
    g_hip_err = "packed weights: " + std::to_string(n) + " bytes, this context's plan packs " + std::to_string(c->blob_floats * sizeof(float));
    return FPC_E_INVALID;
  }
  HIPCHECK(hipSetDevice(c->cfg.device));
  uint32_t h[BLOB_HEADER_FLOATS];
  HIPCHECK(hipMemcpy(h, src_dev, sizeof(h), hipMemcpyDeviceToHost));
  if (!check_blob_header(c, h, &g_hip_err)) return FPC_E_INVALID;
  if (src_dev != (const void*)c->blob) {
    c->weights_loaded = false;
    HIPCHECK(hipMemcpy(c->blob, src_dev, n, hipMemcpyDeviceToDevice));
    HIPCHECK(hipDeviceSynchronize());
  }
  c->weights_loaded = true;
  return FPC_OK;
}

int fpc_mark_weights_loaded(fpc_ctx* c) {
  if (!c) return FPC_E_INVALID;
  uint32_t h[BLOB_HEADER_FLOATS];
  HIPCHECK(hipSetDevice(c->cfg.device));
  HIPCHECK(hipMemcpy(h, c->blob, sizeof(h), hipMemcpyDeviceToHost));
  if (!check_blob_header(c, h, &g_hip_err)) {
    c->weights_loaded = false;
    return FPC_E_INVALID;
  }
  c->weights_loaded = true;
  return FPC_OK;
}

uint64_t fpc_plan_hash(const fpc_ctx* c) { return c ? plan_hash(c) : 0; }

int fpc_check_guards(fpc_ctx* c, long long* bad_words) {
  if (!c || !bad_words) return FPC_E_INVALID;
  *bad_words = 0;
  if (!c->guard_zones || c->guards.empty()) return FPC_E_INVALID;
  HIPCHECK(hipSetDevice(c->cfg.device));
  HIPCHECK(hipDeviceSynchronize());
  unsigned long long* d = nullptr;
  HIPCHECK(hipMalloc((void**)&d, sizeof(*d)));
  {
    const hipError_t e0 = hipMemset(d, 0, sizeof(*d));
    if (e0 != hipSuccess) hipFree(d);
    HIPCHECK(e0);
  }
  count_zones(c, c->slab, c->guards, d);
  count_zones(c, c->bank_slab, c->bank_guards, d);
  count_zones(c, c->topk_slab, c->topk_guards, d);
  count_zones(c, c->pnp_slab, c->pnp_guards, d);
  count_zones(c, c->lm_slab, c->lm_guards, d);
  unsigned long long h = 0;
  const hipError_t e1 = hipStreamSynchronize(c->stream);
  const hipError_t e2 = hipMemcpy(&h, d, sizeof(h), hipMemcpyDeviceToHost);
  hipFree(d);
  HIPCHECK(e1);
  HIPCHECK(e2);
  *bad_words = (long long)h;
  return FPC_OK;
}

namespace {
typedef int (*nccl_bcast_fn)(const void*, void*, size_t, int, int, void*, hipStream_t);
typedef int (*nccl_rank_fn)(void*, int*);
struct RcclApi {
  nccl_bcast_fn bcast = nullptr;
  nccl_rank_fn user_rank = nullptr;
  bool tried = false;
};
static RcclApi g_rccl;
static bool load_rccl() {
  if (g_rccl.tried) return g_rccl.bcast && g_rccl.user_rank;
  g_rccl.tried = true;
  void* h = nullptr;
  void* f = dlsym(RTLD_DEFAULT, "ncclBroadcast");
  if (!f) {
    h = dlopen("librccl.so.1", RTLD_NOW | RTLD_GLOBAL);
    if (!h) h = dlopen("librccl.so", RTLD_NOW | RTLD_GLOBAL);
    if (!h) return false;
    f = dlsym(h, "ncclBroadcast");
  }
  g_rccl.bcast = reinterpret_cast<nccl_bcast_fn>(f);
  void* r = h ? dlsym(h, "ncclCommUserRank") : dlsym(RTLD_DEFAULT, "ncclCommUserRank");
  g_rccl.user_rank = reinterpret_cast<nccl_rank_fn>(r);
  return g_rccl.bcast && g_rccl.user_rank;
}
// ... 1277 lines not shown
      for (int i = 0; i < c->Hc; ++i) f = std::max(f, rm[(size_t)b * c->Hc + i]);
      max_logit[b] = f;
    }
    if (max_desc) { memcpy(&f, w + RANGE_MAX_DESC, 4); max_desc[b] = f; }
    if (nonfinite_input) nonfinite_input[b] = (int32_t)w[RANGE_BAD_INPUT];
  }
  return FPC_OK;
}

int fpc_get_keypoints(fpc_ctx* c, int frame, int cap, int32_t* xy, float* conf, float* desc) {
  if (!c || frame < 0 || frame >= c->B || cap < 0) return FPC_E_INVALID;
  HIPCHECK(hipSetDevice(c->cfg.device));
  HIPCHECK(hipStreamSynchronize(c->stream));
  int32_t k = 0;
  HIPCHECK(hipMemcpy(&k, c->count + frame, sizeof(k), hipMemcpyDeviceToHost));
  if (k > cap || k > c->cap) return FPC_E_CAPACITY;
  if (k == 0) return 0;
  if (xy) HIPCHECK(hipMemcpy(xy, c->xy + (size_t)frame * c->cap * 2, sizeof(int32_t) * 2 * k, hipMemcpyDeviceToHost));
  if (conf) HIPCHECK(hipMemcpy(conf, c->conf + (size_t)frame * c->cap, sizeof(float) * k, hipMemcpyDeviceToHost));
  if (desc) {
    if (!c->cfg.descriptor_enabled) return FPC_E_INVALID;
    HIPCHECK(hipMemcpy(desc, c->desc_out + (size_t)frame * c->cap * c->D, sizeof(float) * c->D * k, hipMemcpyDeviceToHost));
  }
  return k;
}

int fpc_set_timing(fpc_ctx* c, int enable) {
  if (!c) return FPC_E_INVALID;
  c->timing_every = enable > 0 ? enable : 0;
  c->timing_calls = 0;
  c->timing = enable != 0;
  c->timings.clear();
  c->events_used = 0;
  return FPC_OK;
}

int fpc_get_timings(fpc_ctx* c, int cap, const char** names, const char** kernels, float* ms, double* flops,
                    double* mfma_flops, double* bytes) {
  if (!c) return FPC_E_INVALID;
  const int n = (int)c->timings.size();
  for (int i = 0; i < n && i < cap; ++i) {
    const Timing& t = c->timings[i];
    float v = 0.f;
    if (hipEventElapsedTime(&v, t.start, t.stop) != hipSuccess) v = -1.f;
    const Op* op = t.op >= 0 ? &c->ops[t.op] : nullptr;
    if (names) names[i] = op ? op->name.c_str() : "?";
    if (kernels) {
      const char* k = "?";
      if (op) switch (op->type) {
          case OP_STEM: k = c->bf16 ? "stem_bf16_kernel" : c->split ? "stem_pool_x3_kernel" : c->stem2 ? "stem_pool2_kernel" : c->fuse_stem_pool ? "stem_pool_kernel" : "stem_kernel"; break;
          case OP_POOL: k = "maxpool_kernel"; break;
          case OP_CONV: k = op->lean ? lean_kind(op->kind)->symbol : g_kinds[op->kind].symbol; break;
          case OP_BLOCK: k = g_bkinds[op->bkind].symbol; break;
          case OP_WBLOCK: k = g_wkinds[op->wkind].symbol; break;
          case OP_BF16: k = g_fkinds[op->fkind].symbol; break;
          case OP_SOFTMAX: k = "softmax_d2s_kernel"; break;
          case OP_NMS: k = c->nms_one_workgroup ? "nms_rounds_kernel+nms_sort_kernel" : "nms_rounds_kernel+nms_finish_kernel+nms_chunk_sort_kernel+nms_merge_kernel"; break;
          case OP_DESC: k = "descriptor16_kernel"; break;
          case OP_VCONV0: k = "vgg_conv0_kernel"; break;
          case OP_POOL2: k = "maxpool2_kernel"; break;
          case OP_L2NORM: k = "l2norm256_kernel"; break;
        }
      kernels[i] = k;
    }
    if (ms) ms[i] = v;
    if (flops) flops[i] = op ? op->flops_per_frame * t.frames : 0.0;
    if (mfma_flops) mfma_flops[i] = op ? op->mfma_flops_per_frame * t.frames : 0.0;
    if (bytes) bytes[i] = op ? op->bytes_per_frame * t.frames : 0.0;
  }
  return n;
}

}
```

feature-point-cnn_amd/csrc/wblock36_mfma.h:

```cpp
#pragma once
#include <type_traits>
#include <utility>

#include "wblock16_mfma.h"

namespace fpc {

template <int... I, class F>
__device__ __forceinline__ void fpc_static_for_impl(std::integer_sequence<int, I...>, F&& f) {
  (f(std::integral_constant<int, I>{}), ...);
}
template <int N, class F>
__device__ __forceinline__ void fpc_static_for(F&& f) {
  fpc_static_for_impl(std::make_integer_sequence<int, N>{}, f);
}

struct W36Dust {
  static constexpr int W2ROW = 0, W2COL = 64, WPCOL = 144, B1 = 400, B2 = 401, UIN64 = 404, UIN = 448, UOUT = 448 + 4 * 36 * 16;
  static constexpr int floats(int nchunk) { return UOUT + nchunk * 36 * 16; }
};

template <int NB_, int TYT_, int TXT_, bool DUST_ = false>
struct W36Cfg {
  static constexpr int NB = NB_, TYT = TYT_, TXT = TXT_;
// ... 29 lines not shown

template <bool AG0, bool AG1, bool LAST_IN_ASM = false>
__device__ __forceinline__ void fpc_mfma_step(f32x4& c0, f32x4& c1, const f32x4& a0, const f32x4& a1, const f32x4& b0, const f32x4& b1) {
#define FPC_MFMA7                                                                                                      \
  "v_mfma_f32_16x16x4_f32 %0, %2, %10, %0\n\tv_mfma_f32_16x16x4_f32 %1, %6, %14, %1\n\t"                                \
  "v_mfma_f32_16x16x4_f32 %0, %3, %11, %0\n\tv_mfma_f32_16x16x4_f32 %1, %7, %15, %1\n\t"                                \
  "v_mfma_f32_16x16x4_f32 %0, %4, %12, %0\n\tv_mfma_f32_16x16x4_f32 %1, %8, %16, %1\n\t"                                \
  "v_mfma_f32_16x16x4_f32 %0, %5, %13, %0\n\t"
#define FPC_MFMA8 FPC_MFMA7 "v_mfma_f32_16x16x4_f32 %1, %9, %17, %1"
#define FPC_MFMA8_IN                                                                                                   \
  "v"(a0[0]), "v"(a0[1]), "v"(a0[2]), "v"(a0[3]), "v"(a1[0]), "v"(a1[1]), "v"(a1[2]), "v"(a1[3]), "v"(b0[0]), "v"(b0[1]), \
      "v"(b0[2]), "v"(b0[3]), "v"(b1[0]), "v"(b1[1]), "v"(b1[2]), "v"(b1[3])
  if constexpr (LAST_IN_ASM) {
    if constexpr (AG0 && AG1) asm volatile(FPC_MFMA8 : "+a"(c0), "+a"(c1) : FPC_MFMA8_IN);
    else if constexpr (AG0) asm volatile(FPC_MFMA8 : "+a"(c0), "+v"(c1) : FPC_MFMA8_IN);
    else if constexpr (AG1) asm volatile(FPC_MFMA8 : "+v"(c0), "+a"(c1) : FPC_MFMA8_IN);
    else asm volatile(FPC_MFMA8 : "+v"(c0), "+v"(c1) : FPC_MFMA8_IN);
  } else {
    if constexpr (AG0 && AG1) asm volatile(FPC_MFMA7 "s_nop 1" : "+a"(c0), "+a"(c1) : FPC_MFMA8_IN);
    else if constexpr (AG0) asm volatile(FPC_MFMA7 "s_nop 1" : "+a"(c0), "+v"(c1) : FPC_MFMA8_IN);
    else if constexpr (AG1) asm volatile(FPC_MFMA7 "s_nop 1" : "+v"(c0), "+a"(c1) : FPC_MFMA8_IN);
    else asm volatile(FPC_MFMA7 "s_nop 1" : "+v"(c0), "+v"(c1) : FPC_MFMA8_IN);
    c1 = __builtin_amdgcn_mfma_f32_16x16x4f32(a1[3], b1[3], c1, 0, 0, 0);
  }
#undef FPC_MFMA7
#undef FPC_MFMA8
#undef FPC_MFMA8_IN
}

#define W36_MARKER 0x7fffff00

template <bool AG>
__device__ __forceinline__ void fpc_mfma_step16(f32x4& c00, f32x4& c01, f32x4& c10, f32x4& c11, const f32x4& a0, const f32x4& a1,
                                                const f32x4& b00, const f32x4& b01, const f32x4& b10, const f32x4& b11) {
#define FPC_MFMA16                                                                                                      \
  "v_mfma_f32_16x16x4_f32 %0, %4, %12, %0\n\tv_mfma_f32_16x16x4_f32 %1, %4, %16, %1\n\t"                               \
  "v_mfma_f32_16x16x4_f32 %2, %8, %20, %2\n\tv_mfma_f32_16x16x4_f32 %3, %8, %24, %3\n\t"                               \
  "v_mfma_f32_16x16x4_f32 %0, %5, %13, %0\n\tv_mfma_f32_16x16x4_f32 %1, %5, %17, %1\n\t"                               \
  "v_mfma_f32_16x16x4_f32 %2, %9, %21, %2\n\tv_mfma_f32_16x16x4_f32 %3, %9, %25, %3\n\t"                               \
  "v_mfma_f32_16x16x4_f32 %0, %6, %14, %0\n\tv_mfma_f32_16x16x4_f32 %1, %6, %18, %1\n\t"                               \
  "v_mfma_f32_16x16x4_f32 %2, %10, %22, %2\n\tv_mfma_f32_16x16x4_f32 %3, %10, %26, %3\n\t"                             \
  "v_mfma_f32_16x16x4_f32 %0, %7, %15, %0\n\tv_mfma_f32_16x16x4_f32 %1, %7, %19, %1\n\t"                               \
  "v_mfma_f32_16x16x4_f32 %2, %11, %23, %2\n\tv_mfma_f32_16x16x4_f32 %3, %11, %27, %3"
#define FPC_MFMA16_IN                                                                                                   \
  "v"(a0[0]), "v"(a0[1]), "v"(a0[2]), "v"(a0[3]), "v"(a1[0]), "v"(a1[1]), "v"(a1[2]), "v"(a1[3]), "v"(b00[0]), "v"(b00[1]), \
      "v"(b00[2]), "v"(b00[3]), "v"(b01[0]), "v"(b01[1]), "v"(b01[2]), "v"(b01[3]), "v"(b10[0]), "v"(b10[1]), "v"(b10[2]),  \
      "v"(b10[3]), "v"(b11[0]), "v"(b11[1]), "v"(b11[2]), "v"(b11[3])
  if constexpr (AG) asm volatile(FPC_MFMA16 : "+a"(c00), "+a"(c01), "+a"(c10), "+a"(c11) : FPC_MFMA16_IN);
  else asm volatile(FPC_MFMA16 : "+v"(c00), "+v"(c01), "+v"(c10), "+v"(c11) : FPC_MFMA16_IN);
#undef FPC_MFMA16
#undef FPC_MFMA16_IN
}

template <int NB, int TYT, int TXT, bool DUST>
__device__ __forceinline__ void wblock36_body(const WBlockArgs& a) {
  using C = W36Cfg<NB, TYT, TXT, DUST>;
  constexpr int NT = C::NT, TH = C::TH, TW = C::TW, HW = C::HW, HH = C::HH, HROW = C::HROW, HIT = C::HIT;
  constexpr int N = C::N, RH = C::RH, RX = C::RX, RING = C::RING, STEPS = C::STEPS, HPX = C::HPX;
  extern __shared__ __attribute__((aligned(16))) float lds[];
  f32x4* const lds4 = reinterpret_cast<f32x4*>(lds);
  constexpr int TL4 = C::OFF_H0 / 4;

  const int tid = threadIdx.x, lane = tid & 63;
  const unsigned lane16 = (unsigned)lane * 16u;
  const int wave = __builtin_amdgcn_readfirstlane(tid >> 6);
  const int tiles = a.tiles_x * a.tiles_y;
  const int nchunk = a.nchunk;
  const float4* const w1h = a.w1 + (size_t)blockIdx.y * (a.ysplit_floats / 4);
  const float* const b1h = a.b1 + (size_t)blockIdx.y * a.ysplit_floats;

  const bool xcd_order = a.xcd_order && (gridDim.x & 7) == 0;
  const int wg_step = xcd_order ? (int)(gridDim.x >> 3) : (int)gridDim.x;
  const int xchunk = (a.total + 7) >> 3;
  const int wg_first = xcd_order ? (int)(blockIdx.x & 7) * xchunk + (int)(blockIdx.x >> 3) : (int)blockIdx.x;
  const int wg_end = xcd_order ? min(a.total, ((int)(blockIdx.x & 7) + 1) * xchunk) : a.total;
  if (wg_first >= wg_end) return;

  const __amdgpu_buffer_rsrc_t xrsrc = __builtin_amdgcn_make_buffer_rsrc(const_cast<float*>(a.x), 0, (int)a.x_bytes, 0x00020000);
  int okoff[HIT];
  int okoff64[DUST ? C::HIT64 : 1];
  struct TilePos { int b, ty, tx, live; };
  auto tile_pos = [&](int wg) {
    TilePos q;
    q.live = wg < wg_end;
    const int wgc = q.live ? wg : wg_first;
    const int bl = wgc / tiles;
    const int t = wgc - bl * tiles;
    q.b = a.frame0 + bl;
    q.ty = t / a.tiles_x;
    q.tx = t - q.ty * a.tiles_x;
    return q;
  };
  auto halo_base = [&](const TilePos& q) {
    return __builtin_amdgcn_readfirstlane(((q.b * a.H + q.ty * TH) * a.W + q.tx * TW) * a.csx * 4);
  };
  auto halo_tile = [&](const TilePos& q) {
    int tl = tid;
    asm volatile("" : "+v"(tl));
    const int iy0 = q.ty * TH - 1, ix0 = q.tx * TW - 1;
    const int hlim = q.live ? a.H : 0;
#pragma unroll
    for (int i = 0; i < HIT; ++i) {
      const int e = tl + i * NT;
      const int pix = (e * 13108) >> 16, c4 = e - pix * 5;
      const int hy = HW == 18 ? (pix * 3641) >> 16 : (pix * 1928) >> 16;
      const int hx = pix - hy * HW;
      const bool ok = ((unsigned)(iy0 + hy) < (unsigned)hlim) & ((unsigned)(ix0 + hx) < (unsigned)a.W) & (hy < HH) & (c4 < 4);
      const int off = (((hy - 1) * a.W + (hx - 1)) * a.csx + c4 * 4) * 4;
      okoff[i] = ok ? off : W36_MARKER;
    }
    if constexpr (DUST) {
#pragma unroll
      for (int i = 0; i < C::HIT64; ++i) {
        const int pix = tl + i * NT;
        const int hy = HW == 18 ? (pix * 3641) >> 16 : (pix * 1928) >> 16;
        const int hx = pix - hy * HW;
        const bool ok = ((unsigned)(iy0 + hy) < (unsigned)hlim) & ((unsigned)(ix0 + hx) < (unsigned)a.W) & (hy < HH) & (a.dust_in != 0);
        okoff64[i] = ok ? (((hy - 1) * a.W + (hx - 1)) * a.csx + 64) * 4 : W36_MARKER;
      }
    }
  };
  auto load_halo = [&](int base, int hoff) {
#pragma unroll
    for (int i = 0; i < HIT; ++i) {
      int voff;
      asm("v_add_i32 %0, %1, %2 clamp" : "=v"(voff) : "v"(okoff[i]), "s"(base));
      __builtin_amdgcn_raw_ptr_buffer_load_lds(xrsrc, (__attribute__((address_space(3))) void*)(lds + hoff + (i * NT + wave * 64) * 4), 16, voff, 0, 0, 0);
    }
  };
  auto load_halo64 = [&](int base) {
    if constexpr (DUST) {
#pragma unroll
      for (int i = 0; i < C::HIT64; ++i) {
        int voff;
        asm("v_add_i32 %0, %1, %2 clamp" : "=v"(voff) : "v"(okoff64[i]), "s"(base));
        __builtin_amdgcn_raw_ptr_buffer_load_lds(xrsrc, (__attribute__((address_space(3))) void*)(lds + C::D_H64 + (i * NT + wave * 64) * 4), 16, voff, 0, 0, 0);
      }
    }
  };
  const int wt_t = tid >> 4, ch_t = tid & 15;
  const int m_t = ((wt_t & 7) >> 1) * 4 + (wt_t >> 3) * 2 + (wt_t & 1);
  const int trd = ((4 * (wt_t / TXT)) * HW + 4 * (wt_t % TXT)) * HROW + ch_t;
  const int twr = m_t * 16 + ((((ch_t >> 2) ^ (2 * ((m_t >> 3) & 1))) << 2) | (ch_t & 3));
  typedef float f32x2 __attribute__((ext_vector_type(2)));
  f32x2 tp[6][3];
  auto t_read = [&](int rd, int i, int j) { tp[i][j >> 1][j & 1] = lds[rd + (i * HW + j) * HROW]; };
  auto bt6 = [&](f32x2& x0, f32x2& x1, f32x2& x2, f32x2& x3, f32x2& x4, f32x2& x5) {
    const f32x2 k4 = {4.f, 4.f}, km4 = {-4.f, -4.f}, k5 = {-5.f, -5.f}, k2 = {2.f, 2.f}, km2 = {-2.f, -2.f};
    const f32x2 p = __builtin_elementwise_fma(km4, x2, x4), q = __builtin_elementwise_fma(km4, x1, x3);
    const f32x2 r = x4 - x2, s = x3 - x1;
    const f32x2 y0 = __builtin_elementwise_fma(k4, x0, __builtin_elementwise_fma(k5, x2, x4));
    const f32x2 y5 = __builtin_elementwise_fma(k4, x1, __builtin_elementwise_fma(k5, x3, x5));
    x0 = y0;
    x1 = p + q;
    x2 = p - q;
    x3 = __builtin_elementwise_fma(k2, s, r);
    x4 = __builtin_elementwise_fma(km2, s, r);
    x5 = y5;
  };
  auto t_burst = [&]() {
#pragma unroll
    for (int jj = 0; jj < 3; ++jj) bt6(tp[0][jj], tp[1][jj], tp[2][jj], tp[3][jj], tp[4][jj], tp[5][jj]);
// ... 1 lines not shown
    for (int ii = 0; ii < 3; ++ii)
#pragma unroll
      for (int jj = 0; jj < 3; ++jj) {
        const f32x2 ra = tp[2 * ii][jj], rb = tp[2 * ii + 1][jj];
        tp[2 * ii][jj] = __builtin_shufflevector(ra, rb, 0, 2);
        tp[2 * ii + 1][jj] = __builtin_shufflevector(ra, rb, 1, 3);
      }
#pragma unroll
    for (int ii = 0; ii < 3; ++ii) bt6(tp[2 * ii][0], tp[2 * ii + 1][0], tp[2 * ii][1], tp[2 * ii + 1][1], tp[2 * ii][2], tp[2 * ii + 1][2]);
  };
  auto t_write = [&](int wr, int i, int j) { lds[wr + (i * 6 + j) * 256] = tp[2 * (i >> 1) + (j & 1)][j >> 1][i & 1]; };
  auto transform_all = [&](int hoff, int voff) {
#pragma unroll
    for (int i = 0; i < 6; ++i)
#pragma unroll
      for (int j = 0; j < 6; ++j) t_read(trd + hoff, i, j);
    t_burst();
#pragma unroll
    for (int i = 0; i < 6; ++i)
#pragma unroll
      for (int j = 0; j < 6; ++j) t_write(twr + voff, i, j);
  };

  const int aoff4 = (lane & 15) * 4 + ((lane >> 4) ^ (2 * ((lane & 15) >> 3)));
  const unsigned gstride = ((unsigned)nchunk * 36u + (unsigned)C::WPAD) * 1024u;
  const __amdgpu_buffer_rsrc_t wrsrc = __builtin_amdgcn_make_buffer_rsrc(const_cast<float4*>(w1h), 0, (int)(4u * (unsigned)NB * gstride), 0x00020000);
  const unsigned wlane = (unsigned)(wave * NB) * gstride + lane16;
  const int gs_s = __builtin_amdgcn_readfirstlane((int)gstride);
  struct BF { f32x4 v[2][NB]; };
  auto ldb = [&](int s) {
    BF r;
#pragma unroll
    for (int q = 0; q < 2; ++q)
#pragma unroll
      for (int nb = 0; nb < NB; ++nb)
        r.v[q][nb] = __builtin_bit_cast(f32x4, __builtin_amdgcn_raw_buffer_load_b128(wrsrc, (int)wlane, (2 * s + q) * 1024 + nb * gs_s, 0));
    return r;
  };

  [[maybe_unused]] int d_va = 0, d_ua = 0;
  [[maybe_unused]] const __amdgpu_buffer_rsrc_t drsrc =
      DUST ? __builtin_amdgcn_make_buffer_rsrc(const_cast<float*>(a.dust + W36Dust::UOUT), 0, nchunk * 36 * 16 * 4, 0x00020000) : xrsrc;
  [[maybe_unused]] f32x4 du[9];
  [[maybe_unused]] float dacc[9];
  if constexpr (DUST) {
    d_va = wave * 64 + lane;
    d_ua = wave * 64 + 16 * ((lane & 3) ^ (2 * (lane >> 5)));
    for (int i = tid; i < 448 / 4; i += NT) lds4[C::D_HEAD / 4 + i] = reinterpret_cast<const f32x4*>(a.dust)[i];
    for (int i = tid; i < 2304 / 4; i += NT) lds4[C::D_UIN / 4 + i] = reinterpret_cast<const f32x4*>(a.dust + W36Dust::UIN)[i];
  }

  TilePos pos_cur = tile_pos(wg_first);
  int base_cur = halo_base(pos_cur);
  halo_tile(pos_cur);
  load_halo64(base_cur);
  load_halo(base_cur, C::OFF_H0);
  load_halo(base_cur + 64, C::OFF_H1);
  asm volatile("s_waitcnt vmcnt(%0)" ::"n"(HIT) : "memory");
  FPC_LDS_BARRIER();
  transform_all(C::OFF_H0, C::OFF_V0);
  FPC_LDS_BARRIER();

  constexpr int C4 = N / 4, EIT = HPX * C4 / NT, PPI = NT / C4;
  constexpr int CPR = TW / PPI;
  const __amdgpu_buffer_rsrc_t orsrc = __builtin_amdgcn_make_buffer_rsrc(a.out + blockIdx.y * N, 0, W36_MARKER, 0x00020000);

  const int g2s = __builtin_amdgcn_readfirstlane(((a.k8_h + a.k8_x) / 2 + C::WPAD2) * 64);
  const __amdgpu_buffer_rsrc_t w2rsrc = __builtin_amdgcn_make_buffer_rsrc(const_cast<float4*>(a.w2), 0, a.conv_only ? 0 : 4 * NB * g2s * 16, 0x00020000);
  const unsigned w2lane = (unsigned)(wave * NB * g2s) * 16u + lane16;

  const int wg_stamp = wg_first + 2 * wg_step < wg_end ? wg_first + 2 * wg_step : wg_first;
  for (int wg = wg_first; wg < wg_end; wg += wg_step) {
    const int b = pos_cur.b, ty = pos_cur.ty, tx = pos_cur.tx;
    const TilePos pos_next = tile_pos(wg + wg_step);
    const int base_next = halo_base(pos_next);
    if (wg == wg_stamp) { FPC_STAMP(0) FPC_RSTAMP(6) }

    f32x4 acc[36][NB];
    {
      float zf = 0.f;
      asm volatile("" : "+v"(zf));
#pragma unroll
      for (int p = 0; p < 36; ++p)
#pragma unroll
        for (int nb = 0; nb < NB; ++nb) acc[p][nb] = f32x4{zf, zf, zf, zf};
    }

    BF bq[RING];
#pragma unroll
    for (int i = 0; i < RING - 1; ++i) bq[i] = ldb(i);
    if constexpr (DUST) {
      float zf = 0.f;
      asm volatile("" : "+v"(zf));
#pragma unroll
      for (int i = 0; i < 9; ++i) dacc[i] = zf;
    }

    auto chunk_body = [&](auto PAR, const int c) {
      constexpr int par = decltype(PAR)::value;
      constexpr int VB_OFF = par ? C::OFF_V1 : C::OFF_V0, VN_OFF = par ? C::OFF_V0 : C::OFF_V1;
      constexpr int HS_OFF = par ? C::OFF_H1 : C::OFF_H0;
      constexpr int HN_OFF = par ? C::OFF_H0 : C::OFF_H1;
      const int c3 = c + 2;
      const bool nxt = c3 >= nchunk;
      const int l_base = (nxt ? base_next : base_cur) + (nxt ? c3 - nchunk : c3) * 64;
      int ao = aoff4 + VB_OFF / 4, trd_c = trd + HN_OFF, twr_c = twr + VN_OFF;
      asm volatile("" : "+v"(ao), "+v"(trd_c), "+v"(twr_c));
      [[maybe_unused]] int dva = d_va + VB_OFF / 4;
      [[maybe_unused]] f32x4 dv[3];
      if constexpr (DUST) asm volatile("" : "+v"(dva));
      constexpr int AQ = 2;
      f32x4 ac[2][AQ];
#pragma unroll
      for (int q = 0; q < AQ; ++q) ac[0][q] = lds4[ao + q * 64];
#ifdef FPC_DIAG_STEPS
      unsigned long long tq[11] = {0, 0, 0, 0, 0, 0, 0, 0, 0, 0, 0};
#define FPC_TQ(i) asm volatile("s_memtime %0" : "=s"(tq[i]));
#else
#define FPC_TQ(i)
#endif
      fpc_static_for<STEPS>([&](auto S) __attribute__((always_inline)) {
        constexpr int s = decltype(S)::value;
        if constexpr (s % 2 == 0) { FPC_TQ(s / 2) }
        bq[(s + RING - 1) % RING] = ldb(c * STEPS + s + RING - 1);
        if (s + 1 < STEPS) {
#pragma unroll
          for (int q = 0; q < AQ; ++q) ac[(s + 1) & 1][q] = lds4[ao + ((s + 1) * AQ + q) * 64];
        }
        constexpr int SPS = 36 / STEPS;
#pragma unroll
        for (int u = 0; u < SPS; ++u) {
          const int slot = s * SPS + u;
          if (slot == 1) {
            if (c3 == nchunk) halo_tile(pos_next);
            load_halo(l_base, HS_OFF);
          } else if (slot >= 2 && slot < 14) {
#pragma unroll
            for (int k = 0; k < 3; ++k) { const int e = (slot - 2) * 3 + k; t_read(trd_c, e / 6, e % 6); }
          } else if (slot == 14) {
            t_burst();
          } else if (slot >= 15 && slot < 33) {
#pragma unroll
            for (int k = 0; k < 2; ++k) { const int e = (slot - 15) * 2 + k; t_write(twr_c, e / 6, e % 6); }
          }
          if constexpr (DUST) {
            auto dread = [&](int i0) {
#pragma unroll
              for (int k = 0; k < 3; ++k) dv[k] = lds4[dva + (i0 + k) * 256];
            };
            auto dfma = [&](int i0) {
#pragma unroll
              for (int k = 0; k < 3; ++k)
#pragma unroll
                for (int e = 0; e < 4; ++e) dacc[i0 + k] = __builtin_fmaf(dv[k][e], du[i0 + k][e], dacc[i0 + k]);
            };
            if (slot == 3) {
#pragma unroll
              for (int i = 0; i < 9; ++i)
                du[i] = __builtin_bit_cast(f32x4, __builtin_amdgcn_raw_buffer_load_b128(drsrc, d_ua + i * 256, c * (36 * 16 * 4), 0));
            } else if (slot == 23) {
              dread(0);
            } else if (slot == 25) {
              dfma(0);
              dread(3);
            } else if (slot == 27) {
              dfma(3);
              dread(6);
            } else if (slot == 29) {
              dfma(6);
            }
          }
        }
        __builtin_amdgcn_sched_barrier(0);
        {
          const BF& bv = bq[s % RING];
          constexpr int p0 = 2 * s, p1 = 2 * s + 1;
          if constexpr (NB == 2)
            fpc_mfma_step16<(p0 < C::PAG)>(acc[p0][0], acc[p0][1], acc[p1][0], acc[p1][1], ac[s & 1][0], ac[s & 1][1], bv.v[0][0], bv.v[0][1],
                                           bv.v[1][0], bv.v[1][NB - 1]);
          else
            fpc_mfma_step<true, true>(acc[p0][0], acc[p1][0], ac[s & 1][0], ac[s & 1][1], bv.v[0][0], bv.v[1][0]);
        }
        __builtin_amdgcn_sched_barrier(0);
      });
      FPC_TQ(9)
      asm volatile("s_waitcnt vmcnt(%0)" ::"n"(2 * NB * (RING - 1)) : "memory");
// ... 387 lines not shown
              acc2[mb][nb][r] = __builtin_bit_cast(float, __builtin_amdgcn_raw_buffer_load_b32(xrsrc, xl + so + 64 * nb, 0, 0));
          }
        if constexpr (DUST) {
#pragma unroll
          for (int mb = 0; mb < 8; ++mb)
#pragma unroll
            for (int r = 0; r < 4; ++r) acc2[mb][0][r] = __builtin_fmaf(dhv[mb][r], dw2r, acc2[mb][0][r]);
        }
        gemm_over(RH / 4, KH, 0);
        if (wg == wg_stamp && half == 0) { FPC_STAMP(3) }
      }

      if (wg == wg_stamp && half == 0) { FPC_STAMP(4) }
      asm volatile("s_nop 15\n\ts_nop 7" ::: "memory");
      FPC_LDS_BARRIER();
      {
        int ew = C::OFF_H0 + (4 * kq) * RH + 16 * (wave * NB) + n16;
        asm volatile("" : "+v"(ew));
#pragma unroll
        for (int nb = 0; nb < NB; ++nb) {
          const float bias = a.b2[16 * (wave * NB + nb) + n16];
#pragma unroll
          for (int mb = 0; mb < 8; ++mb)
#pragma unroll
            for (int r = 0; r < 4; ++r) lds[ew + 16 * nb + (16 * mb + r) * RH] = acc2[mb][nb][r] + bias;
        }
      }
      FPC_LDS_BARRIER();
      store_out();
      if constexpr (DUST) {
        const bool b3 = (dq & 8) != 0, b2 = (dq & 4) != 0, b1 = (dq & 2) != 0;
        float r1[4], r2[2];
#pragma unroll
        for (int k = 0; k < 4; ++k) r1[k] = (b3 ? dpart[4 + k] : dpart[k]) + __shfl_xor(b3 ? dpart[k] : dpart[4 + k], 8);
#pragma unroll
        for (int k = 0; k < 2; ++k) r2[k] = (b2 ? r1[2 + k] : r1[k]) + __shfl_xor(b2 ? r1[k] : r1[2 + k], 4);
        float tot = (b1 ? r2[1] : r2[0]) + __shfl_xor(b1 ? r2[0] : r2[1], 2);
        tot += __shfl_xor(tot, 1);
        const int dpx = 32 * wave + 4 * (dq >> 1) + dpxl, dhf = dq & 1, drow = dpx / TW, dcol = dpx % TW;
        tot += dx64 + lds[C::D_HEAD + W36Dust::B2];
        tot = tot > 0.f ? tot : 0.f;
        const bool ok = (drow < rows_valid) & (x0 + dcol < a.W);
        const int doff = ok ? ((drow * a.W + dcol) * a.cso + 64 + 4 * dhf) * 4 : W36_MARKER;
        int voff;
        asm("v_add_i32 %0, %1, %2 clamp" : "=v"(voff) : "v"(doff), "s"(obase));
        const f32x4 v = {dhf ? 0.f : tot, 0.f, 0.f, 0.f};
        __builtin_amdgcn_raw_buffer_store_b128(__builtin_bit_cast(__attribute__((__vector_size__(4 * sizeof(unsigned)))) unsigned, v), orsrc, voff, 0, 0);
      }
      if (wg == wg_stamp && half == 0) { FPC_STAMP(5) FPC_RSTAMP(7) }
      FPC_LDS_BARRIER();
    }
    pos_cur = pos_next;
    base_cur = base_next;
  }
}

template <int NB, int TYT, int TXT>
__global__ __launch_bounds__(256, 1) void wblock36_kernel(const WBlockArgs a) {
  wblock36_body<NB, TYT, TXT, false>(a);
}

template <int TYT, int TXT>
__global__ __launch_bounds__(256, 1) void wblock36_dust_kernel(const WBlockArgs a) {
  wblock36_body<1, TYT, TXT, true>(a);
}

}
```

feature-point-cnn_amd/csrc/wblock36p_mfma.h:

```cpp
#pragma once
#include "wblock36_mfma.h"

namespace fpc {

template <int TYT_, int TXT_, bool DUST_ = false>
struct W36PCfg {
  static constexpr int TYT = TYT_, TXT = TXT_;
  static constexpr bool DUST = DUST_;
  static_assert(TYT * TXT == 16 && (TYT == 4 || TYT == 2), "16 Winograd tiles per workgroup tile: 4 x 4 or 2 x 8");
  static constexpr int NT = 512, NTH = 256, NPOS = 36, KC = 16, N = 64;
  static constexpr int TH = 4 * TYT, TW = 4 * TXT, HH = TH + 2, HW = TW + 2, NHALO = HH * HW;
  static constexpr int HROW = 20;
  static constexpr int HIT = (NHALO * 5 + NTH - 1) / NTH;
  static constexpr int HALO_FLOATS = HIT * NTH * 4;
  static constexpr int V_FLOATS = NPOS * 16 * 16;
  static constexpr int OFF_V0 = 0, OFF_H1 = V_FLOATS, OFF_H0 = OFF_H1 + HALO_FLOATS, OFF_V1 = OFF_H0 + HALO_FLOATS;
  static constexpr int RH = N + 8;
  static constexpr int PX = TH * TW;
  static constexpr int T_FLOATS = PX * RH;
  static constexpr int BASE_FLOATS = (OFF_V1 + V_FLOATS) > (OFF_H0 + T_FLOATS) ? (OFF_V1 + V_FLOATS) : (OFF_H0 + T_FLOATS);
  static constexpr int HIT64 = (NHALO + NTH - 1) / NTH;
  static constexpr int D_HEAD = BASE_FLOATS, D_COL = D_HEAD + 64, D_UIN = D_HEAD + 448, D_V64 = D_UIN + 2304, D_M64 = D_V64 + 576, D_H64 = D_M64 + 576;
  static constexpr int LDS_FLOATS = DUST ? D_H64 + HIT64 * NTH * 4 : BASE_FLOATS;
  static constexpr int LDS_BYTES = LDS_FLOATS * 4;
  static_assert(LDS_BYTES <= 160 * 1024, "LDS");
  static constexpr int STEPS = 9;
  static constexpr int WPAD = W36Cfg<1, TYT, TXT>::WPAD, WPAD2 = W36Cfg<1, TYT, TXT>::WPAD2;
  static_assert(WPAD >= 36, "a wave prefetches up to one chunk past its stream's end");
};

template <int TYT, int TXT, int RING, bool DUST>
__device__ __forceinline__ void wblock36p_body(const WBlockArgs& a) {
  using C = W36PCfg<TYT, TXT, DUST>;
  constexpr int TH = C::TH, TW = C::TW, HW = C::HW, HH = C::HH, HROW = C::HROW, HIT = C::HIT, NTH = C::NTH;
  constexpr int N = C::N, RH = C::RH, STEPS = C::STEPS, PX = C::PX;
  static_assert(STEPS % RING == 0 && RING >= 2, "ring slots must line up across chunks");
  extern __shared__ __attribute__((aligned(16))) float lds[];
  f32x4* const lds4 = reinterpret_cast<f32x4*>(lds);
  constexpr int TL4 = C::OFF_H0 / 4;

  const int tid = threadIdx.x, lane = tid & 63;
  const unsigned lane16 = (unsigned)lane * 16u;
  const int wave = __builtin_amdgcn_readfirstlane(tid >> 6);
  const int grp = wave & 3;
  const int hs = wave >> 2;
  const int tiles = a.tiles_x * a.tiles_y;
  const int nchunk = a.nchunk;
  const float4* const w1h = a.w1 + (size_t)blockIdx.y * (a.ysplit_floats / 4);
  const float* const b1h = a.b1 + (size_t)blockIdx.y * a.ysplit_floats;

  const bool xcd_order = a.xcd_order && (gridDim.x & 7) == 0;
  const int wg_step = xcd_order ? (int)(gridDim.x >> 3) : (int)gridDim.x;
  const int xchunk = (a.total + 7) >> 3;
  const int wg_first = xcd_order ? (int)(blockIdx.x & 7) * xchunk + (int)(blockIdx.x >> 3) : (int)blockIdx.x;
  const int wg_end = xcd_order ? min(a.total, ((int)(blockIdx.x & 7) + 1) * xchunk) : a.total;
  if (wg_first >= wg_end) return;

  const __amdgpu_buffer_rsrc_t xrsrc = __builtin_amdgcn_make_buffer_rsrc(const_cast<float*>(a.x), 0, (int)a.x_bytes, 0x00020000);
  struct TilePos { int b, ty, tx, live; };
  auto tile_pos = [&](int wg) {
    TilePos q;
    q.live = wg < wg_end;
    const int wgc = q.live ? wg : wg_first;
    const int bl = wgc / tiles;
    const int t = wgc - bl * tiles;
    q.b = a.frame0 + bl;
    q.ty = t / a.tiles_x;
    q.tx = t - q.ty * a.tiles_x;
    return q;
  };
  auto halo_base = [&](const TilePos& q) {
    return __builtin_amdgcn_readfirstlane(((q.b * a.H + q.ty * TH) * a.W + q.tx * TW) * a.csx * 4);
  };
  constexpr bool KEEP_HYX = !DUST;
  auto slot_hyx = [&](int tl, int i) {
    const int e = tl + i * NTH;
    const int pix = (e * 13108) >> 16, c4 = e - pix * 5;
    const int hy = HW == 18 ? (pix * 3641) >> 16 : (pix * 1928) >> 16;
    const int hx = pix - hy * HW;
    const bool slot_ok = (hy < HH) & (c4 < 4);
    return slot_ok ? (hy << 16) | (c4 << 8) | hx : 0x7fff0000;
  };
  int okoff[HIT];
  [[maybe_unused]] int hyx[KEEP_HYX ? HIT : 1];
  if (hs == 1) {
    const int tl = tid & (NTH - 1);
#pragma unroll
    for (int i = 0; i < HIT; ++i) {
      if constexpr (KEEP_HYX) hyx[i] = slot_hyx(tl, i);
      okoff[i] = W36_MARKER;
    }
  }
  [[maybe_unused]] int okoff64[C::HIT64];
  auto slot_hyx64 = [&](int tl, int i) {
    const int pix = tl + i * NTH;
    const int hy = HW == 18 ? (pix * 3641) >> 16 : (pix * 1928) >> 16;
    const int hx = pix - hy * HW;
    return (hy < HH && a.dust_in) ? (hy << 16) | hx : 0x7fff0000;
  };
  if constexpr (DUST) {
    if (hs == 1) {
#pragma unroll
      for (int i = 0; i < C::HIT64; ++i) okoff64[i] = W36_MARKER;
    }
  }
  auto halo_tile = [&](const TilePos& q) {
    const int iy0 = q.ty * TH - 1, ix0 = q.tx * TW - 1;
    const int hlim = q.live ? a.H : 0;
    int tlq = tid & (NTH - 1);
    asm volatile("" : "+v"(tlq));
#pragma unroll
    for (int i = 0; i < HIT; ++i) {
      int hv = KEEP_HYX ? hyx[KEEP_HYX ? i : 0] : slot_hyx(tlq, i);
      asm volatile("" : "+v"(hv));
      const int hy = hv >> 16, hx = hv & 0xff, c4 = (hv >> 8) & 0xff;
      const bool ok = ((unsigned)(iy0 + hy) < (unsigned)hlim) & ((unsigned)(ix0 + hx) < (unsigned)a.W);
      okoff[i] = ok ? (((hy - 1) * a.W + (hx - 1)) * a.csx + c4 * 4) * 4 : W36_MARKER;
    }
    if constexpr (DUST) {
#pragma unroll
      for (int i = 0; i < C::HIT64; ++i) {
        int hv = slot_hyx64(tlq, i);
        asm volatile("" : "+v"(hv));
        const int hy = hv >> 16, hx = hv & 0xffff;
        const bool ok = ((unsigned)(iy0 + hy) < (unsigned)hlim) & ((unsigned)(ix0 + hx) < (unsigned)a.W);
        okoff64[i] = ok ? (((hy - 1) * a.W + (hx - 1)) * a.csx + 64) * 4 : W36_MARKER;
      }
    }
  };
  auto load_halo64 = [&](int base) {
    if constexpr (DUST) {
#pragma unroll
      for (int i = 0; i < C::HIT64; ++i) {
        int voff;
        asm("v_add_i32 %0, %1, %2 clamp" : "=v"(voff) : "v"(okoff64[i]), "s"(base));
        __builtin_amdgcn_raw_ptr_buffer_load_lds(xrsrc, (__attribute__((address_space(3))) void*)(lds + C::D_H64 + (i * NTH + grp * 64) * 4), 16, voff, 0, 0, 0);
      }
    }
  };
  auto load_halo = [&](int base, int hoff_f) {
#pragma unroll
    for (int i = 0; i < HIT; ++i) {
      int voff;
      asm("v_add_i32 %0, %1, %2 clamp" : "=v"(voff) : "v"(okoff[i]), "s"(base));
      __builtin_amdgcn_raw_ptr_buffer_load_lds(xrsrc, (__attribute__((address_space(3))) void*)(lds + hoff_f + (i * NTH + grp * 64) * 4), 16, voff, 0, 0, 0);
    }
  };
  const int tq = tid & (NTH - 1);
  const int wt_t = tq >> 4, ch_t = tq & 15;
// ... 338 lines not shown
          if (tid_t < 16) {
            float mm[36];
#pragma unroll
            for (int p = 0; p < 36; ++p) mm[p] = lds[C::D_M64 + p * 16 + tid_t];
            const float bias64 = lds[C::D_HEAD + W36Dust::B1];
            float tt[4][6];
#pragma unroll
            for (int j = 0; j < 6; ++j) {
              const float m0 = mm[0 * 6 + j], m1 = mm[1 * 6 + j], m2 = mm[2 * 6 + j], m3 = mm[3 * 6 + j], m4 = mm[4 * 6 + j], m5 = mm[5 * 6 + j];
              const float s12 = m1 + m2, d12 = m1 - m2, s34 = m3 + m4, d34 = m3 - m4;
              tt[0][j] = m0 + s12 + s34;
              tt[1][j] = __builtin_fmaf(2.f, d34, d12);
              tt[2][j] = __builtin_fmaf(4.f, s34, s12);
              tt[3][j] = __builtin_fmaf(8.f, d34, d12) + m5;
            }
            const int T = 8 * ((tid_t >> 1) & 1) + 2 * (tid_t >> 2) + (tid_t & 1);
            const int hb = C::OFF_H0 + ((4 * (T / TXT)) * TW + 4 * (T % TXT)) * RH + 64;
#pragma unroll
            for (int i = 0; i < 4; ++i) {
              const float m0 = tt[i][0], m1 = tt[i][1], m2 = tt[i][2], m3 = tt[i][3], m4 = tt[i][4], m5 = tt[i][5];
              const float s12 = m1 + m2, d12 = m1 - m2, s34 = m3 + m4, d34 = m3 - m4;
              float yv64[4];
              yv64[0] = m0 + s12 + s34 + bias64;
              yv64[1] = __builtin_fmaf(2.f, d34, d12) + bias64;
              yv64[2] = __builtin_fmaf(4.f, s34, s12) + bias64;
              yv64[3] = __builtin_fmaf(8.f, d34, d12) + m5 + bias64;
#pragma unroll
              for (int jj = 0; jj < 4; ++jj) lds[hb + (i * TW + jj) * RH] = yv64[jj] > 0.f ? yv64[jj] : 0.f;
            }
          }
        }
      }
      FPC_LDS_BARRIER();
    };
    if (hs == 0) out_transform(std::integral_constant<int, 0>{});
    else out_transform(std::integral_constant<int, 1>{});
    if (wg == wg_stamp) { FPC_STAMP(2) }

    const int y0 = ty * TH, x0 = tx * TW;
    const int rows_valid = min(TH, a.H - y0);
    const int xbase = __builtin_amdgcn_readfirstlane(((b * a.H + y0) * a.W + x0) * a.csx * 4);
    const int obase = __builtin_amdgcn_readfirstlane(((b * a.H + y0) * a.W + x0) * a.cso * 4);
    const int m0 = tid_t / C4, c4t = tid_t - m0 * C4;
    const int rsub = __builtin_amdgcn_readfirstlane(m0 / TW), pcol = m0 % TW;
    const int ocol = (x0 + pcol < a.W) ? (pcol * a.cso + c4t * 4) * 4 : W36_MARKER;
    int erd = TL4 + m0 * (RH / 4) + c4t;
    asm volatile("" : "+v"(erd));
    auto store_out = [&]() {
#pragma unroll
      for (int i = 0; i < EIT; ++i) {
        const int prow = i * RPI + rsub;
        if (prow < rows_valid) {
          f32x4 v = lds4[erd + i * PPI * (RH / 4)];
          if (!a.conv_only) {
            v.x = v.x > 0.f ? v.x : 0.f;
            v.y = v.y > 0.f ? v.y : 0.f;
            v.z = v.z > 0.f ? v.z : 0.f;
            v.w = v.w > 0.f ? v.w : 0.f;
          }
          int voff;
          const int so = obase + prow * a.W * a.cso * 4;
          asm("v_add_i32 %0, %1, %2 clamp" : "=v"(voff) : "v"(ocol), "s"(so));
          __builtin_amdgcn_raw_buffer_store_b128(__builtin_bit_cast(__attribute__((__vector_size__(4 * sizeof(unsigned)))) unsigned, v), orsrc, voff, 0, 0);
        }
      }
    };

    if (a.conv_only) {
      store_out();
      FPC_LDS_BARRIER();
    } else {
      f32x4 acc2[8];
      const int pb = hs;
      [[maybe_unused]] float dpart[8];
      [[maybe_unused]] float dw2r = 0.f;
      [[maybe_unused]] float dhv[8][4];
      [[maybe_unused]] const int dq = lane_t & 15, dpxl = lane_t >> 4;
      [[maybe_unused]] float dx64 = 0.f;
      if constexpr (DUST) {
        if (!proj) {
          const int px = 32 * wave + 4 * (dq >> 1) + dpxl;
          dx64 = __builtin_bit_cast(float, __builtin_amdgcn_raw_buffer_load_b32(xrsrc, (((px / TW) * a.W + px % TW) * a.csx + 64) * 4, xbase, 0));
        }
        const f32x4 wq = lds4[C::D_COL / 4 + dq];
        const float w64 = dq == 0 ? lds[C::D_COL + 64] : 0.f;
#pragma unroll
        for (int it = 0; it < 8; ++it) {
          const int px = 32 * wave + 4 * it + dpxl;
          const f32x4 hq = lds4[TL4 + px * (RH / 4) + dq];
          const float h64 = lds[C::OFF_H0 + px * RH + 64];
          float v = h64 * w64;
#pragma unroll
          for (int e = 0; e < 4; ++e) v = __builtin_fmaf(hq[e], wq[e], v);
          dpart[it] = v;
        }
        dw2r = lds[C::D_HEAD + W36Dust::W2ROW + 16 * grp + n16];
#pragma unroll
        for (int mb = 0; mb < 8; ++mb)
#pragma unroll
          for (int r = 0; r < 4; ++r) dhv[mb][r] = lds[C::OFF_H0 + (128 * pb + 16 * mb + 4 * kq + r) * RH + 64];
      }
      auto ldb2 = [&](int s) {
        return __builtin_bit_cast(f32x4, __builtin_amdgcn_raw_buffer_load_b128(w2rsrc, (int)w2lane, s * 1024, 0));
      };
      constexpr int KH = N / 16;
      auto gemm_over = [&](int ksteps, int s_first) {
        int ar = TL4 + (128 * pb + n16) * (RH / 4) + kq;
        asm volatile("" : "+v"(ar));
        f32x4 cb[4];
#pragma unroll
        for (int i = 0; i < 3; ++i) cb[i] = ldb2(s_first + i);
        f32x4 af[2][2];
#pragma unroll
        for (int q = 0; q < 2; ++q) af[0][q] = lds4[ar + q * 16 * (RH / 4)];
        for (int g = 0; g < ksteps; g += 4) {
#pragma unroll
          for (int u = 0; u < 4; ++u) {
            cb[(u + 3) & 3] = ldb2(s_first + g + u + 3);
            fpc_static_for<4>([&](auto B_) __attribute__((always_inline)) {
              constexpr int blk = decltype(B_)::value;
              if (blk + 1 < 4) {
#pragma unroll
                for (int q = 0; q < 2; ++q) af[(blk + 1) & 1][q] = lds4[ar + (g + u) * 4 + ((blk + 1) * 2 + q) * 16 * (RH / 4)];
              } else {
// ... 80 lines not shown
            for (int r = 0; r < 4; ++r) acc2[mb][r] = __builtin_fmaf(dhv[mb][r], dw2r, acc2[mb][r]);
        }
        gemm_over(KH, 0);
        if (wg == wg_stamp) { FPC_STAMP(3) }
      }

      if (wg == wg_stamp) { FPC_STAMP(4) }
      asm volatile("s_nop 15\n\ts_nop 7" ::: "memory");
      FPC_LDS_BARRIER();
      {
        int ew = C::OFF_H0 + (128 * pb + 4 * kq) * RH + 16 * grp + n16;
        asm volatile("" : "+v"(ew));
        const float bias = a.b2[16 * grp + n16];
#pragma unroll
        for (int mb = 0; mb < 8; ++mb)
#pragma unroll
          for (int r = 0; r < 4; ++r) lds[ew + (16 * mb + r) * RH] = acc2[mb][r] + bias;
      }
      FPC_LDS_BARRIER();
      store_out();
      if constexpr (DUST) {
        const bool b3 = (dq & 8) != 0, b2 = (dq & 4) != 0, b1 = (dq & 2) != 0;
        float r1[4], r2[2];
#pragma unroll
        for (int k = 0; k < 4; ++k) r1[k] = (b3 ? dpart[4 + k] : dpart[k]) + __shfl_xor(b3 ? dpart[k] : dpart[4 + k], 8);
#pragma unroll
        for (int k = 0; k < 2; ++k) r2[k] = (b2 ? r1[2 + k] : r1[k]) + __shfl_xor(b2 ? r1[k] : r1[2 + k], 4);
        float tot = (b1 ? r2[1] : r2[0]) + __shfl_xor(b1 ? r2[0] : r2[1], 2);
        tot += __shfl_xor(tot, 1);
        const int dpx = 32 * wave + 4 * (dq >> 1) + dpxl, dhf = dq & 1, drow = dpx / TW, dcol = dpx % TW;
        tot += dx64 + lds[C::D_HEAD + W36Dust::B2];
        tot = tot > 0.f ? tot : 0.f;
        const bool ok = (drow < rows_valid) & (x0 + dcol < a.W);
        const int doff = ok ? ((drow * a.W + dcol) * a.cso + 64 + 4 * dhf) * 4 : W36_MARKER;
        int voff;
        asm("v_add_i32 %0, %1, %2 clamp" : "=v"(voff) : "v"(doff), "s"(obase));
        const f32x4 v = {dhf ? 0.f : tot, 0.f, 0.f, 0.f};
        __builtin_amdgcn_raw_buffer_store_b128(__builtin_bit_cast(__attribute__((__vector_size__(4 * sizeof(unsigned)))) unsigned, v), orsrc, voff, 0, 0);
      }
      if (wg == wg_stamp) { FPC_STAMP(5) FPC_RSTAMP(7) }
      FPC_LDS_BARRIER();
    }
    pos_cur = pos_next;
    base_cur = base_next;
  }
}

template <int TYT, int TXT, int RING = 3>
__global__ __launch_bounds__(512, 1) void wblock36p_kernel(const WBlockArgs a) {
  wblock36p_body<TYT, TXT, RING, false>(a);
}

template <int TYT, int TXT, int RING = 3>
__global__ __launch_bounds__(512, 1) void wblock36p_dust_kernel(const WBlockArgs a) {
  wblock36p_body<TYT, TXT, RING, true>(a);
}

}
```

feature-point-cnn_amd/csrc/wblock_mfma.h:

```cpp
#pragma once
#include "block_mfma.h"

namespace fpc {

struct WBlockArgs {
  const float* x;
  int csx, nchunk;
  int H, W;
  const float4* w1;
  const float* b1;
  const float4* w2;
  const float* b2;
  int k8_h, k8_x;
  float* out;
  int cso, tiles_x, tiles_y, frame0;
  int total;
  int xcd_order;
  int ysplit_floats;
  unsigned x_bytes;
  int conv_only;
  const float* dust;
  int dust_in;
#ifdef FPC_DIAG
  unsigned long long* stamps;
#endif
};

template <int KC, int NBT, int CMID_>
struct WBlockCfg {
  static constexpr int TH = 8, TW = 16, NT = 512;
  static constexpr int HW = TW + 2, HH = TH + 2;
  static constexpr int ROW4 = KC / 4 + 1;
  static constexpr int CMID = CMID_;
  static constexpr int ROWH4 = CMID / 4 + 1;
  static constexpr int HALO_BYTES = HH * HW * ROW4 * 16;
  static constexpr int V_BYTES = 16 * 32 * ROW4 * 16;
  static constexpr int M_BYTES = 16 * 32 * 36 * 4;
  static constexpr int H_BYTES = 128 * ROWH4 * 16;
  static constexpr int LDS_BYTES = (HALO_BYTES + V_BYTES) > (M_BYTES + H_BYTES) ? (HALO_BYTES + V_BYTES) : (M_BYTES + H_BYTES);
  static constexpr int GN = NBT >= 4 ? 2 : 1;
  static constexpr int GX = 8 / GN;
  static constexpr int PX = 16 / GX;
  static constexpr int NBW = NBT / GN;
};

__device__ __forceinline__ float4 fpc_ldg_su(const float4* ubase, unsigned lane_bytes) {
  typedef const char __attribute__((address_space(1))) * gptr;
  typedef float f4v __attribute__((ext_vector_type(4)));
  gptr b = (gptr) reinterpret_cast<const char*>(ubase);
  asm("" : "+s"(b));
  const f4v v = *reinterpret_cast<const f4v __attribute__((address_space(1)))*>(b + lane_bytes);
  return make_float4(v.x, v.y, v.z, v.w);
}

template <int KC, int NBT, int CMID_>
__global__ __launch_bounds__(512, 2) void wblock_mfma_kernel(const WBlockArgs a) {
  using C = WBlockCfg<KC, NBT, CMID_>;
  constexpr int NT = C::NT, TH = C::TH, TW = C::TW, HW = C::HW, HH = C::HH, ROW4 = C::ROW4, K8 = KC / 8, KC4 = KC / 4;
  constexpr int NV = HH * HW * KC4, ITER = (NV + NT - 1) / NT, ROWH4 = C::ROWH4, CMID = C::CMID;
  constexpr int GN = C::GN, PX = C::PX, NBW = C::NBW;
  extern __shared__ float4 lds4[];
  float4* halo4 = lds4;
  float4* v4 = lds4 + C::HALO_BYTES / 16;

  const int tid = threadIdx.x, lane = tid & 63;
  const unsigned lane16 = (unsigned)lane * 16u;
  const int wave = __builtin_amdgcn_readfirstlane(tid >> 6);
  const int gx = wave / GN, gn = wave % GN;
  const int half = lane >> 5, l31 = lane & 31;
  const int tiles = a.tiles_x * a.tiles_y;
  FPC_STAMP(0)

  float4 stage[ITER];
  auto load_chunk = [&](int wg, int chunk) {
    const int bl = wg / tiles;
// ... 370 lines not shown
```

include/fpc.h:

```cpp
#ifndef FPC_H
#define FPC_H

#include <stddef.h>
#include <stdint.h>

#ifdef __cplusplus
extern "C" {
#endif

#define FPC_ABI_VERSION 4
#define FPC_PACK_LAYOUT_REVISION 4

enum {
  FPC_OK = 0,
  FPC_E_INVALID = -1,
  FPC_E_NO_DEVICE = -2,
  FPC_E_HIP = -3,
  FPC_E_NO_WEIGHTS = -4,
  FPC_E_MISSING_KEY = -5,
  FPC_E_CAPACITY = -6,
  FPC_E_NOT_CONVERGED = -7,
  FPC_E_RANGE = -8,
  FPC_E_NONFINITE = -9
};


enum { FPC_F32 = 0, FPC_BF16 = 1, FPC_F32_SPLIT = 2, FPC_F32_SPLIT_F16 = 3 };
enum { FPC_ARCH_RESNET = 0, FPC_ARCH_VGG = 1 };

typedef struct fpc_config {
  int device;
  int height, width;
  int max_batch;
  int cell;
  int nms_dist;
  float conf_thresh;
  int border_remove;
  int descriptor_enabled;
  int max_keypoints;
  int in_channels;
  int dtype;
  int arch;
  int num_streams;
  unsigned plan_flags;
  int nms_round_launches;
  int min_sub_batch;
} fpc_config;

enum {
  FPC_PLAN_NO_FUSED_BLOCKS = 1 << 0,
  FPC_PLAN_NO_WINOGRAD = 1 << 1,
  FPC_PLAN_NO_WINOGRAD_DETECTOR = 1 << 2,
  FPC_PLAN_NO_WINOGRAD_LAYER_IN1 = 1 << 3,
  FPC_PLAN_NO_XCD_ORDER = 1 << 4,
  FPC_PLAN_NO_FUSED_STEM_POOL = 1 << 5,
  FPC_PLAN_SPLIT_HEADS = 1 << 6,
  FPC_PLAN_NMS_IN_LINE = 1 << 7,
  FPC_PLAN_NO_PERSISTENT_GRID = 1 << 8,
  FPC_PLAN_LAYER1_TILE_8x16 = 1 << 9,
  FPC_PLAN_WINOGRAD_GEN1 = 1 << 10,
  FPC_PLAN_NO_LATENCY_TILES = 1 << 11,
  FPC_PLAN_NMS_ONE_WORKGROUP = 1 << 12,
  FPC_PLAN_NO_FUSED_SOFTMAX = 1 << 13,
  FPC_PLAN_WINOGRAD_GEN2 = 1 << 14,
  FPC_PLAN_HEADS_IN_LINE = 1 << 17,
  FPC_PLAN_DETECTOR_GEN1 = 1 << 16,
  FPC_PLAN_W36_ONE_WAVE = 1 << 18,
  FPC_PLAN_STEM_ROUND3 = 1 << 20,
  FPC_PLAN_CONV_ROUND1 = 1 << 21,
  FPC_PLAN_CONVT_PHASES = 1 << 19,
  FPC_PLAN_GUARD_ZONES = 1 << 15
};

typedef struct fpc_tensor {
  const char* name;
  const float* data;
  int ndim;
  int64_t shape[4];
} fpc_tensor;

typedef struct fpc_device_results {
  const int32_t* count;
  const int32_t* n_candidates;
  const int32_t* xy;
  const float* conf;
  const float* desc;
  int capacity;
  int desc_dim;
} fpc_device_results;

typedef struct fpc_ctx fpc_ctx;

int fpc_abi_version(void);
const char* fpc_build_flags(void);
const char* fpc_strerror(int code);
const char* fpc_last_hip_error(void);

int fpc_default_config(fpc_config* cfg);

int fpc_create(fpc_ctx** out, const fpc_config* cfg);
void fpc_destroy(fpc_ctx* ctx);

int fpc_load_weights(fpc_ctx* ctx, const fpc_tensor* tensors, int n);

size_t fpc_packed_size(const fpc_ctx* ctx);
void* fpc_packed_device_ptr(fpc_ctx* ctx);
int fpc_export_packed(fpc_ctx* ctx, void* host_dst, size_t cap);
int fpc_import_packed(fpc_ctx* ctx, const void* host_src, size_t n);
int fpc_import_packed_device(fpc_ctx* ctx, const void* dev_src, size_t n);
int fpc_mark_weights_loaded(fpc_ctx* ctx);
uint64_t fpc_plan_hash(const fpc_ctx* ctx);
int fpc_pack_layout_revision(void);

int fpc_check_guards(fpc_ctx* ctx, long long* bad_words);

int fpc_broadcast_weights(fpc_ctx* ctx, void* nccl_comm, int root);

int fpc_set_stream(fpc_ctx* ctx, void* hip_stream);
void* fpc_get_stream(fpc_ctx* ctx);
void* fpc_upload_stream(fpc_ctx* ctx);
typedef struct fpc_stream_report_t {
  int n_streams;
  int slot[16], queue[16];
  int probing;
  int hw_queues_found;
  int process_probe_rounds, process_probe_launches, process_inconclusive_rounds;
  float process_probe_ms;
  int create_probe_rounds;
  float create_placement_ms;
  int process_registered_streams;
} fpc_stream_report_t;
int fpc_stream_report(fpc_ctx* ctx, fpc_stream_report_t* out);
int fpc_sync(fpc_ctx* ctx);

int fpc_forward(fpc_ctx* ctx, const float* frames_dev, int n, float* prob_map_dev,
                float* desc_dev, float* logits_dev);

int fpc_read_activation(fpc_ctx* ctx, const char* name, int frame0, int n, float* out_dev, int* channels, int* height,
                        int* width);

int fpc_detect(fpc_ctx* ctx, const float* frames_dev, int n);

enum { FPC_U8_GRAY = 0, FPC_U8_RGB_HWC = 1, FPC_U8_BGR_HWC = 2, FPC_U8_BGR_HWC_GRAY = 3 };
int fpc_detect_u8(fpc_ctx* ctx, const uint8_t* frames_dev, int n, int layout);
int fpc_detect_u8_resized(fpc_ctx* ctx, const uint8_t* frames_dev, int n, int src_h, int src_w, int layout);
const float* fpc_u8_staging(fpc_ctx* ctx);

int fpc_homography_adaptation(fpc_ctx* ctx, const float* frames_dev, int n, const float* homographies_host,
                              const float* inverses_host, int num, int erosion_radius, int aggregation,
                              float* prob_out_dev);

int fpc_get_points(fpc_ctx* ctx, const float* prob_map_dev, const float* desc_nchw_dev, int n);

int fpc_sample_descriptors(fpc_ctx* ctx, const float* desc_nchw_dev, const double* xy_dev, int k, float* out_dev);

int fpc_match(fpc_ctx* ctx, const float* q_dev, int nq, const float* t_dev, int nt, int cross_check,
              float max_dist, int32_t* match_dev, float* dist_dev);
int fpc_first_within(fpc_ctx* ctx, const float* key_dev, int nk, const float* cur_dev, int nc,
                     float tolerance, int32_t* first_dev);

enum { FPC_PAIR_KEY = 0, FPC_PAIR_PREVIOUS = 1 };
int fpc_match_frames(fpc_ctx* ctx, int n, int pairing, const float* key_dev, const int32_t* nkey_dev,
                     int cross_check, float max_dist, float ratio, int32_t* match_dev, float* dist_dev);
int fpc_first_within_frames(fpc_ctx* ctx, int n, const float* key_dev, const int32_t* nkey_dev,
                            float tolerance, int32_t* first_dev);
// ... 139 lines not shown
```

Baseline: 12090.

## Add tile-shape round: stacked-frame W36 tiles, 8x2 conv tiles, 4x16 block

Result: faster. 12380, median of 6 (+2.4%).

```diff
diff --git a/feature-point-cnn_amd/_lib.py b/feature-point-cnn_amd/_lib.py
--- a/feature-point-cnn_amd/_lib.py
+++ b/feature-point-cnn_amd/_lib.py
@@ -16,7 +16,7 @@
     "fpc_get_counts", "fpc_get_keypoints", "fpc_set_timing", "fpc_get_timings", "fpc_match", "fpc_first_within",
     "fpc_detect_u8", "fpc_u8_staging", "fpc_homography_adaptation", "fpc_detect_u8_resized",
     "fpc_sample_descriptors", "fpc_plan_hash", "fpc_broadcast_weights", "fpc_read_activation",
-    "fpc_pack_layout_revision", "fpc_check_guards", "fpc_stream_report", "fpc_output_range",
+    "fpc_pack_layout_revision", "fpc_tile_choice", "fpc_check_guards", "fpc_stream_report", "fpc_output_range",
     "fpc_match_frames", "fpc_first_within_frames",
     "fpc_default_ransac_params", "fpc_ransac_homography", "fpc_homography_frames",
     "fpc_bank_create", "fpc_bank_destroy", "fpc_bank_get", "fpc_bank_store", "fpc_bank_store_rows", "fpc_bank_clear",
@@ -40,6 +40,7 @@
     "no_xcd_order": 1 << 4, "no_fused_stem_pool": 1 << 5, "split_heads": 1 << 6, "nms_in_line": 1 << 7,
     "no_persistent_grid": 1 << 8, "layer1_tile_8x16": 1 << 9, "winograd_gen1": 1 << 10, "no_latency_tiles": 1 << 11,
     "nms_one_workgroup": 1 << 12, "no_fused_softmax": 1 << 13, "winograd_gen2": 1 << 14, "guard_zones": 1 << 15, "detector_gen1": 1 << 16, "heads_in_line": 1 << 17, "w36_one_wave": 1 << 18, "convt_phases": 1 << 19, "stem_round3": 1 << 20, "conv_round1": 1 << 21,
+    "tiles_round5": 1 << 22,
 }
 
 
@@ -219,6 +220,7 @@
     l.fpc_plan_hash.restype = ctypes.c_uint64
     l.fpc_broadcast_weights.argtypes = [vp, vp, ci]
     l.fpc_pack_layout_revision.restype = ci
+    l.fpc_tile_choice.argtypes = [ci, ci, ci, ci, ctypes.c_uint]
     l.fpc_check_guards.argtypes = [vp, ctypes.POINTER(ctypes.c_longlong)]
     l.fpc_stream_report.argtypes = [vp, ctypes.POINTER(FpcStreamReport)]
     l.fpc_set_timing.argtypes = [vp, ci]
diff --git a/feature-point-cnn_amd/csrc/fpc_api.hip b/feature-point-cnn_amd/csrc/fpc_api.hip
--- a/feature-point-cnn_amd/csrc/fpc_api.hip
+++ b/feature-point-cnn_amd/csrc/fpc_api.hip
@@ -146,7 +146,8 @@
   X(B320_s2_K32_C256, 3, 20, 2, 32, 1, 4, 2, 2, 256)         \
   X(B310_s2_K32_C256, 3, 10, 2, 32, 1, 4, 1, 2, 256)         \
   X(B320_s2_K32_C128, 3, 20, 2, 32, 1, 4, 2, 1, 128)         \
-  X(B320_s1_K64_C256, 3, 20, 1, 64, 1, 4, 2, 2, 256)
+  X(B320_s1_K64_C256, 3, 20, 1, 64, 1, 4, 2, 2, 256)         \
+  X(B416_s2_K32_C128, 4, 16, 2, 32, 1, 4, 2, 1, 128)
 
 enum BKind {
 #define X(name, ...) BK_##name,
@@ -209,6 +210,11 @@
   X(W36_C65_4x4, 4, 4)    \
   X(W36_C65_2x8, 2, 8)
 
+#define FPC_W36S_KINDS(X) \
+  X(W36S_C128_4x4, 2, 4, 4)
+#define FPC_W36PC_KINDS(X) \
+  X(W36PC_C64_8x2, 8, 2)
+
 enum WKind {
 #define X(name, ...) WK_##name,
   FPC_WBLOCK_KINDS(X)
@@ -217,6 +223,8 @@
   FPC_W36D_KINDS(X)
   FPC_W36P_KINDS(X)
   FPC_W36PD_KINDS(X)
+  FPC_W36S_KINDS(X)
+  FPC_W36PC_KINDS(X)
 #undef X
       WK_COUNT
 };
@@ -276,6 +284,20 @@
     hipLaunchKernelGGL((wblock36p_dust_kernel<TYT, TXT>), grid, dim3(512), lds, st, a);                   \
   }
 FPC_W36PD_KINDS(X)
+#undef X
+#define X(name, NB, TYT, TXT)                                                                             \
+  static void launchw_##name(const WBlockArgs& a, dim3 grid, hipStream_t st) {                            \
+    constexpr int lds = W36Cfg<NB, TYT, TXT>::LDS_BYTES;                                                  \
+    hipLaunchKernelGGL((wblock36s_kernel<NB, TYT, TXT>), grid, dim3(256), lds, st, a);                    \
+  }
+FPC_W36S_KINDS(X)
+#undef X
+#define X(name, TYT, TXT)                                                                                  \
+  static void launchw_##name(const WBlockArgs& a, dim3 grid, hipStream_t st) {                            \
+    constexpr int lds = W36PCfg<TYT, TXT, false, true>::LDS_BYTES;                                        \
+    hipLaunchKernelGGL((wconv36p_kernel<TYT, TXT>), grid, dim3(512), lds, st, a);                         \
+  }
+FPC_W36PC_KINDS(X)
 #undef X
 
 static const WKindInfo g_wkinds[WK_COUNT] = {
@@ -309,6 +331,16 @@
    W36PCfg<TYT, TXT, true>::LDS_BYTES, 4, 4 * TYT, 4 * TXT, 512, (const void*)wblock36p_dust_kernel<TYT, TXT>, launchw_##name, true},
     FPC_W36PD_KINDS(X)
 #undef X
+#define X(name, NB, TYT, TXT)                                                                             \
+  {#name, "wblock36s_kernel<" #NB ", " #TYT ", " #TXT ">", 3, 16, 2 * NB, 64 * NB,                         \
+   W36Cfg<NB, TYT, TXT>::LDS_BYTES, 4 * NB, 4 * TYT, 4 * TXT, 256, (const void*)wblock36s_kernel<NB, TYT, TXT>, launchw_##name},
+    FPC_W36S_KINDS(X)
+#undef X
+#define X(name, TYT, TXT)                                                                                 \
+  {#name, "wconv36p_kernel<" #TYT ", " #TXT ", 3>", 3, 16, 2, 64,                                            \
+   W36PCfg<TYT, TXT, false, true>::LDS_BYTES, 4, 4 * TYT, 4 * TXT, 512, (const void*)wconv36p_kernel<TYT, TXT>, launchw_##name},
+    FPC_W36PC_KINDS(X)
+#undef X
 };
 
 static size_t w1_floats(const WKindInfo& k, int nchunk) {
@@ -333,13 +365,23 @@
   const double t2 = std::ceil((double)tiles * (cout / 128) / cus) * 1.0, t1 = std::ceil((double)tiles * (cout / 64) / cus) * 0.53;
   return t1 < t2 ? 64 : 128;
 }
-static WKind w36_kind(int cout, int H, int W, bool paired = false) {
-  const int t44 = ((H + 15) / 16) * ((W + 15) / 16), t28 = ((H + 7) / 8) * ((W + 31) / 32);
+static WKind w36_kind(int cout, int H, int W, bool paired = false, bool conv82 = false) {
+  const int t44 = ((H + 15) / 16) * ((W + 15) / 16), t28 = ((H + 7) / 8) * ((W + 31) / 32), t82 = ((H + 31) / 32) * ((W + 7) / 8);
+  if (conv82 && cout == 64 && paired && t82 < std::min(t44, t28)) return WK_W36PC_C64_8x2;
   if (cout == 65 && paired) return t28 < t44 ? WK_W36PD_C65_2x8 : WK_W36PD_C65_4x4;
   if (cout == 65) return t28 < t44 ? WK_W36_C65_2x8 : WK_W36_C65_4x4;
   if (cout == 64 && paired) return t28 < t44 ? WK_W36P_C64_2x8 : WK_W36P_C64_4x4;
   if (cout == 64) return t28 < t44 ? WK_W36_C64_2x8 : WK_W36_C64_4x4;
   return t28 < t44 ? WK_W36_C128_2x8 : WK_W36_C128_4x4;
+}
+
+static WKind w36_stacked_kind(WKind wk) { return wk == WK_W36_C128_4x4 || wk == WK_W36_C128_2x8 ? WK_W36S_C128_4x4 : WK_COUNT; }
+static int w36_stacked_rows(int Hf, int W, int frames, WKind sk, int tiles_now) {
+  if (sk == WK_COUNT) return 0;
+  const int th = g_wkinds[sk].TH, tw = g_wkinds[sk].TW;
+  if (Hf % 4 != 0 || Hf < th) return 0;
+  const int rows = (frames * Hf + th - 1) / th;
+  return rows * ((W + tw - 1) / tw) < frames * tiles_now ? rows : 0;
 }
 
 #define FPC_BF16_KINDS(X)                                                                   \
@@ -418,6 +460,7 @@
   BKind bkind = BK_COUNT;
   BlockArgs bargs{};
   WKind wkind = WK_COUNT;
+  int hash_bkind = -1, hash_wkind = -1;
   WBlockArgs wargs{};
   FKind fkind = FK_COUNT;
   BlockBfArgs fargs{};
@@ -446,6 +489,8 @@
   hipEvent_t start, stop;
   int op;
   int frames;
+  int wkind = -1;
+  double mfma_flops = -1.0;
 };
 
 }
@@ -502,6 +547,7 @@
   bool winograd_in1 = true;
   bool winograd_det = true;
   int w36_cus = 0;
+  bool tiles_round6 = true;
   bool w36_paired = true;
   bool winograd_det_gen3 = true;
   bool winograd = true;
@@ -821,8 +867,7 @@
   c->convw.push_back(cw);
 }
 
-static void retile_last(fpc_ctx* c, BKind small) {
-  if (!c->latency_tiles || c->ops.empty() || c->ops.back().type != OP_BLOCK) return;
+static void retile_block(fpc_ctx* c, BKind small) {
   const BKindInfo &k0 = g_bkinds[c->ops.back().bkind], &k = g_bkinds[small];
   if (k.KC != k0.KC || k.WN * k.NB != k0.WN * k0.NB || k.S != k0.S || k.CMIDP != k0.CMIDP) { c->plan_error = true; return; }
   Op& o = c->ops.back();
@@ -835,6 +880,22 @@
   a.tiles_y = (a.Ho + k.TH - 1) / k.TH;
   o.mfma_flops_per_frame = 2.0 * a.tiles_x * a.tiles_y * (k.WM * k.MB * 32.0) * (k.WN * k.NB * 32.0) *
                            ((double)a.nchunk * k.KC * 9 + (a.k8_h + a.k8_x) * 8.0);
+}
+static void retile_last(fpc_ctx* c, BKind small) {
+  if (!c->latency_tiles || c->ops.empty() || c->ops.back().type != OP_BLOCK) return;
+  retile_block(c, small);
+}
+static long block_rows(BKind k, int Ho, int Wo) {
+  const BKindInfo& b = g_bkinds[k];
+  return (long)((Ho + b.TH - 1) / b.TH) * ((Wo + b.TW - 1) / b.TW) * (b.WM * b.MB * 32);
+}
+static void retile_rows(fpc_ctx* c, BKind fit) {
+  if (!c->tiles_round6 || c->ops.empty() || c->ops.back().type != OP_BLOCK) return;
+  Op& o = c->ops.back();
+  if (block_rows(fit, o.bargs.Ho, o.bargs.Wo) >= block_rows(o.bkind, o.bargs.Ho, o.bargs.Wo)) return;
+  const BKind had = o.bkind;
+  retile_block(c, fit);
+  if (!c->plan_error) c->ops.back().hash_bkind = had;
 }
 
 static void retile_last(fpc_ctx* c, Kind small) {
@@ -958,6 +1019,7 @@
             (cout > k.CMID ? ", channels " + std::to_string(n0) + ".." + std::to_string(n0 + k.CMID - 1) : std::string()) + "]";
   op.prefix = prefix;
   op.wkind = wk;
+  if (wk == WK_W36PC_C64_8x2) op.hash_wkind = w36_kind(64, H, W, true);
   op.wconv = true;
   op.plain_conv = !bn;
   op.n0 = n0;
@@ -1666,6 +1728,7 @@
   block("encoder.layer2.0", K_T620_3x3s2_K32_N128, K_T620_1x1_K64_N128, 2, c->x2, 64, 64, 64, H4, W4, c->h8, 128,
         128, 128, c->x3, 128, true, false, BK_B620_s2_K32_C128);
   if (c->fuse_blocks) retile_last(c, BK_B320_s2_K32_C128);
+  if (c->fuse_blocks) retile_rows(c, BK_B416_s2_K32_C128);
   block("encoder.layer2.1", K_T620_3x3_K64_N128, K_T620_1x1_K64_N128, 1, c->x3, 128, 128, 128, Hc, Wc, c->h8, 128,
         128, 128, feat, 256, false, false, BK_B620_s1_K64_C128);
   if (c->fuse_blocks) {
@@ -1712,7 +1775,7 @@
       const bool g3 = c->winograd_gen == 3 && w36_fits(c->B, H16, W16, 256, 256);
       const int in1_parts = g3 ? 4 : 2;
       for (int n0 = 0; n0 < 256; n0 += 256 / in1_parts)
-        add_wconv(c, p, true, g3 ? w36_kind(64, H16, W16, c->w36_paired) : c->winograd_gen >= 2 ? WK_W16_C128 : WK_W816_K32_C128, c->y16a, 256, 256, H16, W16, c->h16, 256, 256, n0, true, &bo);
+        add_wconv(c, p, true, g3 ? w36_kind(64, H16, W16, c->w36_paired, c->tiles_round6) : c->winograd_gen >= 2 ? WK_W16_C128 : WK_W816_K32_C128, c->y16a, 256, 256, H16, W16, c->h16, 256, 256, n0, true, &bo);
       const size_t in1_ops = in1_parts + 1;
       ConvSpec t{};
       t.name = p + ".conv2+bn2+identity+relu";
@@ -1837,7 +1900,8 @@
   mix(c->vconv0_off);
   for (size_t i = 0; i < c->ops.size(); ++i) {
     const Op& op = c->ops[i];
-    mix((uint64_t)op.type); mix((uint64_t)op.kind); mix((uint64_t)op.bkind); mix((uint64_t)op.wkind); mix((uint64_t)op.fkind);
+    mix((uint64_t)op.type); mix((uint64_t)op.kind); mix((uint64_t)(op.hash_bkind >= 0 ? (BKind)op.hash_bkind : op.bkind));
+    mix((uint64_t)(op.hash_wkind >= 0 ? (WKind)op.hash_wkind : op.wkind)); mix((uint64_t)op.fkind);
     mix((uint64_t)(op.phase + 1)); mix((uint64_t)op.n0);
     for (char ch : op.prefix) mix((uint64_t)(unsigned char)ch);
     const fpc_ctx::ConvW& cw = c->convw[i];
@@ -2365,6 +2429,8 @@
   hipStream_t st;
   int frames;
   hipEvent_t s{}, e{};
+  int wkind = -1;
+  double mfma_flops = -1.0;
   LaunchTimer(fpc_ctx* c_, int op_, hipStream_t st_, int frames_) : c(c_), op(op_), st(st_), frames(frames_) {
     if (c->timing) {
       s = next_event(c);
@@ -2375,7 +2441,7 @@
   ~LaunchTimer() {
     if (c->timing) {
       hipEventRecord(e, st);
-      c->timings.push_back({s, e, op, frames});
+      c->timings.push_back({s, e, op, frames, wkind, mfma_flops});
     }
   }
 };
@@ -2494,19 +2560,31 @@
           const int fpl = w36_frames_per_launch(a.H, a.W, a.csx, a.cso);
           const float* x0 = a.x;
           float* o0 = a.out;
+          const int Hf = a.H, tx_f = a.tiles_x, ty_f = a.tiles_y;
+          const WKind sk = c->tiles_round6 ? w36_stacked_kind(op.wkind) : WK_COUNT;
+          double mf = 0.0;
           for (int g0 = 0; g0 < n; g0 += fpl) {
             const int gn = std::min(fpl, n - g0);
             a.frame0 = 0;
-            a.x = x0 + (size_t)(f0 + g0) * a.H * a.W * a.csx;
-            a.out = o0 + (size_t)(f0 + g0) * a.H * a.W * a.cso;
-            a.total = a.tiles_x * a.tiles_y * gn;
-            a.x_bytes = (unsigned)((unsigned long long)gn * a.H * a.W * a.csx * sizeof(float));
+            a.x = x0 + (size_t)(f0 + g0) * Hf * a.W * a.csx;
+            a.out = o0 + (size_t)(f0 + g0) * Hf * a.W * a.cso;
+            a.x_bytes = (unsigned)((unsigned long long)gn * Hf * a.W * a.csx * sizeof(float));
+            const int srows = w36_stacked_rows(Hf, a.W, gn, sk, tx_f * ty_f);
+            const WKind lk = srows ? sk : op.wkind;
+            a.H = srows ? gn * Hf : Hf;
+            a.frame_h = srows ? Hf : 0;
+            a.tiles_x = srows ? (a.W + g_wkinds[sk].TW - 1) / g_wkinds[sk].TW : tx_f;
+            a.tiles_y = srows ? srows : ty_f;
+            a.total = srows ? a.tiles_x * srows : tx_f * ty_f * gn;
+            if (srows) t.wkind = sk;
+            mf += srows ? wkind_mfma_flops(g_wkinds[sk], a.total, a.nchunk, a.k8_h + a.k8_x) : op.mfma_flops_per_frame * gn;
             const int cus_cap = c->w36_cus > 0 ? std::min(c->num_cus, c->w36_cus) : c->num_cus;
             const int cus8 = std::max(1, cus_cap / 8 / std::max(1, op.grid_y)), per_xcd = (a.total + 7) / 8;
             const int rounds = (per_xcd + cus8 - 1) / cus8;
             const int grid3 = 8 * std::min(cus8, (per_xcd + rounds - 1) / rounds);
-            g_wkinds[op.wkind].launch(a, dim3(std::min(a.total, grid3), op.grid_y), sb.st);
+            g_wkinds[lk].launch(a, dim3(std::min(a.total, grid3), op.grid_y), sb.st);
           }
+          if (t.wkind >= 0) t.mfma_flops = mf;
           break;
         }
         g_wkinds[op.wkind].launch(a, dim3(std::min(a.total, grid), op.grid_y), sb.st);
@@ -2910,6 +2988,8 @@
     c->winograd_det_gen3 = !(pf & FPC_PLAN_DETECTOR_GEN1);
     c->w36_paired = !(pf & FPC_PLAN_W36_ONE_WAVE);
     if (const char* e = getenv("FPC_W36_PAIRED")) c->w36_paired = atoi(e) != 0;
+    c->tiles_round6 = !(pf & FPC_PLAN_TILES_ROUND5);
+    if (const char* e = getenv("FPC_TILES_ROUND6")) c->tiles_round6 = atoi(e) != 0;
     if (const char* e = getenv("FPC_W36_CUS")) c->w36_cus = std::max(0, atoi(e));
     if (const char* e = getenv("FPC_WINOGRAD_DET_GEN")) c->winograd_det_gen3 = atoi(e) >= 3;
     c->winograd = !(pf & FPC_PLAN_NO_WINOGRAD);
@@ -3121,6 +3201,24 @@
 
 uint64_t fpc_plan_hash(const fpc_ctx* c) { return c ? plan_hash(c) : 0; }
 
+int fpc_tile_choice(int what, int H, int W, int frames, unsigned plan_flags) {
+  const bool r6 = !(plan_flags & FPC_PLAN_TILES_ROUND5);
+  if (H <= 0 || W <= 0 || frames <= 0) return FPC_E_INVALID;
+  switch (what) {
+    case 0: {
+      const WKindInfo& k = g_wkinds[w36_kind(128, H, W)];
+      return r6 ? w36_stacked_rows(H, W, frames, WK_W36S_C128_4x4, ((H + k.TH - 1) / k.TH) * ((W + k.TW - 1) / k.TW)) : 0;
+    }
+    case 1: { const WKindInfo& k = g_wkinds[w36_kind(64, H, W, true, r6)]; return 100 * k.TH + k.TW; }
+    case 2: {
+      const BKind k5 = BK_B320_s2_K32_C128, k6 = BK_B416_s2_K32_C128;
+      const BKindInfo& k = g_bkinds[r6 && block_rows(k6, H, W) < block_rows(k5, H, W) ? k6 : k5];
+      return 100 * k.TH + k.TW;
+    }
+  }
+  return FPC_E_INVALID;
+}
+
 int fpc_check_guards(fpc_ctx* c, long long* bad_words) {
   if (!c || !bad_words) return FPC_E_INVALID;
   *bad_words = 0;
@@ -4504,7 +4602,7 @@
           case OP_POOL: k = "maxpool_kernel"; break;
           case OP_CONV: k = op->lean ? lean_kind(op->kind)->symbol : g_kinds[op->kind].symbol; break;
           case OP_BLOCK: k = g_bkinds[op->bkind].symbol; break;
-          case OP_WBLOCK: k = g_wkinds[op->wkind].symbol; break;
+          case OP_WBLOCK: k = g_wkinds[t.wkind >= 0 ? t.wkind : op->wkind].symbol; break;
           case OP_BF16: k = g_fkinds[op->fkind].symbol; break;
           case OP_SOFTMAX: k = "softmax_d2s_kernel"; break;
           case OP_NMS: k = c->nms_one_workgroup ? "nms_rounds_kernel+nms_sort_kernel" : "nms_rounds_kernel+nms_finish_kernel+nms_chunk_sort_kernel+nms_merge_kernel"; break;
@@ -4517,7 +4615,7 @@
     }
     if (ms) ms[i] = v;
     if (flops) flops[i] = op ? op->flops_per_frame * t.frames : 0.0;
-    if (mfma_flops) mfma_flops[i] = op ? op->mfma_flops_per_frame * t.frames : 0.0;
+    if (mfma_flops) mfma_flops[i] = !op ? 0.0 : t.mfma_flops >= 0 ? t.mfma_flops : op->mfma_flops_per_frame * t.frames;
     if (bytes) bytes[i] = op ? op->bytes_per_frame * t.frames : 0.0;
   }
   return n;
diff --git a/feature-point-cnn_amd/csrc/wblock36_mfma.h b/feature-point-cnn_amd/csrc/wblock36_mfma.h
--- a/feature-point-cnn_amd/csrc/wblock36_mfma.h
+++ b/feature-point-cnn_amd/csrc/wblock36_mfma.h
@@ -105,9 +105,10 @@
 #undef FPC_MFMA16_IN
 }
 
-template <int NB, int TYT, int TXT, bool DUST>
+template <int NB, int TYT, int TXT, bool DUST, bool STACK = false>
 __device__ __forceinline__ void wblock36_body(const WBlockArgs& a) {
   using C = W36Cfg<NB, TYT, TXT, DUST>;
+  static_assert(!STACK || (!DUST && (C::HH + 1) * C::HW * 5 <= C::HIT * C::NT), "the stacked walk's extra halo row must fit the halo buffer");
   constexpr int NT = C::NT, TH = C::TH, TW = C::TW, HW = C::HW, HH = C::HH, HROW = C::HROW, HIT = C::HIT;
   constexpr int N = C::N, RH = C::RH, RX = C::RX, RING = C::RING, STEPS = C::STEPS, HPX = C::HPX;
   extern __shared__ __attribute__((aligned(16))) float lds[];
@@ -147,20 +148,39 @@
   auto halo_base = [&](const TilePos& q) {
     return __builtin_amdgcn_readfirstlane(((q.b * a.H + q.ty * TH) * a.W + q.tx * TW) * a.csx * 4);
   };
-  auto halo_tile = [&](const TilePos& q) {
+  auto seam_row = [&](const TilePos& q) {
+    if constexpr (STACK) {
+      const int r = (q.ty * TH) % a.frame_h;
+      const int d = r == 0 ? 0 : a.frame_h - r;
+      return d > TH ? -1 : d == 0 ? 0 : d + 1;
+    } else {
+      return -1;
+    }
+  };
+  const int wrow_u = STACK ? __builtin_amdgcn_readfirstlane((tid >> 4) / TXT) : 0;
+  auto seam_shift = [&](int zrow) { return (STACK && zrow > 0 && 4 * wrow_u + 1 >= zrow) ? HW * HROW : 0; };
+  auto halo_tile = [&](const TilePos& q, [[maybe_unused]] int zrow = -1) {
     int tl = tid;
     asm volatile("" : "+v"(tl));
     const int iy0 = q.ty * TH - 1, ix0 = q.tx * TW - 1;
     const int hlim = q.live ? a.H : 0;
+    [[maybe_unused]] const int zs = zrow > 0 ? zrow : 0x7fff, hmax = zrow > 0 ? HH + 1 : HH;
 #pragma unroll
     for (int i = 0; i < HIT; ++i) {
       const int e = tl + i * NT;
       const int pix = (e * 13108) >> 16, c4 = e - pix * 5;
       const int hy = HW == 18 ? (pix * 3641) >> 16 : (pix * 1928) >> 16;
       const int hx = pix - hy * HW;
+      if constexpr (STACK) {
+        const int hys = hy - (hy > zs ? 1 : 0);
+        const bool ok = ((unsigned)(iy0 + hys) < (unsigned)hlim) & ((unsigned)(ix0 + hx) < (unsigned)a.W) & (hy < hmax) & (hy != zrow) & (c4 < 4);
+        const int off = (((hys - 1) * a.W + (hx - 1)) * a.csx + c4 * 4) * 4;
+        okoff[i] = ok ? off : W36_MARKER;
+      } else {
       const bool ok = ((unsigned)(iy0 + hy) < (unsigned)hlim) & ((unsigned)(ix0 + hx) < (unsigned)a.W) & (hy < HH) & (c4 < 4);
       const int off = (((hy - 1) * a.W + (hx - 1)) * a.csx + c4 * 4) * 4;
       okoff[i] = ok ? off : W36_MARKER;
+      }
     }
     if constexpr (DUST) {
 #pragma unroll
@@ -268,13 +288,16 @@
 
   TilePos pos_cur = tile_pos(wg_first);
   int base_cur = halo_base(pos_cur);
-  halo_tile(pos_cur);
+  [[maybe_unused]] int zrow_cur = seam_row(pos_cur);
+  if constexpr (STACK) halo_tile(pos_cur, zrow_cur);
+  else halo_tile(pos_cur);
   load_halo64(base_cur);
   load_halo(base_cur, C::OFF_H0);
   load_halo(base_cur + 64, C::OFF_H1);
   asm volatile("s_waitcnt vmcnt(%0)" ::"n"(HIT) : "memory");
   FPC_LDS_BARRIER();
-  transform_all(C::OFF_H0, C::OFF_V0);
+  if constexpr (STACK) transform_all(C::OFF_H0 + seam_shift(zrow_cur), C::OFF_V0);
+  else transform_all(C::OFF_H0, C::OFF_V0);
   FPC_LDS_BARRIER();
 
   constexpr int C4 = N / 4, EIT = HPX * C4 / NT, PPI = NT / C4;
@@ -290,6 +313,7 @@
     const int b = pos_cur.b, ty = pos_cur.ty, tx = pos_cur.tx;
     const TilePos pos_next = tile_pos(wg + wg_step);
     const int base_next = halo_base(pos_next);
+    [[maybe_unused]] const int zrow_next = seam_row(pos_next);
     if (wg == wg_stamp) { FPC_STAMP(0) FPC_RSTAMP(6) }
 
     f32x4 acc[36][NB];
@@ -321,6 +345,7 @@
       const bool nxt = c3 >= nchunk;
       const int l_base = (nxt ? base_next : base_cur) + (nxt ? c3 - nchunk : c3) * 64;
       int ao = aoff4 + VB_OFF / 4, trd_c = trd + HN_OFF, twr_c = twr + VN_OFF;
+      if constexpr (STACK) trd_c += seam_shift(par && c + 1 >= nchunk ? zrow_next : zrow_cur);
       asm volatile("" : "+v"(ao), "+v"(trd_c), "+v"(twr_c));
       [[maybe_unused]] int dva = d_va + VB_OFF / 4;
       [[maybe_unused]] f32x4 dv[3];
@@ -348,6 +373,8 @@
         for (int u = 0; u < SPS; ++u) {
           const int slot = s * SPS + u;
           if (slot == 1) {
+            if constexpr (STACK) { if (c3 == nchunk) halo_tile(pos_next, zrow_next); }
+            else
             if (c3 == nchunk) halo_tile(pos_next);
             load_halo(l_base, HS_OFF);
           } else if (slot >= 2 && slot < 14) {
@@ -841,6 +868,7 @@
     }
     pos_cur = pos_next;
     base_cur = base_next;
+    if constexpr (STACK) zrow_cur = zrow_next;
   }
 }
 
@@ -849,6 +877,11 @@
   wblock36_body<NB, TYT, TXT, false>(a);
 }
 
+template <int NB, int TYT, int TXT>
+__global__ __launch_bounds__(256, 1) void wblock36s_kernel(const WBlockArgs a) {
+  wblock36_body<NB, TYT, TXT, false, true>(a);
+}
+
 template <int TYT, int TXT>
 __global__ __launch_bounds__(256, 1) void wblock36_dust_kernel(const WBlockArgs a) {
   wblock36_body<1, TYT, TXT, true>(a);
diff --git a/feature-point-cnn_amd/csrc/wblock36p_mfma.h b/feature-point-cnn_amd/csrc/wblock36p_mfma.h
--- a/feature-point-cnn_amd/csrc/wblock36p_mfma.h
+++ b/feature-point-cnn_amd/csrc/wblock36p_mfma.h
@@ -3,11 +3,11 @@
 
 namespace fpc {
 
-template <int TYT_, int TXT_, bool DUST_ = false>
+template <int TYT_, int TXT_, bool DUST_ = false, bool CONV_ = false>
 struct W36PCfg {
   static constexpr int TYT = TYT_, TXT = TXT_;
-  static constexpr bool DUST = DUST_;
-  static_assert(TYT * TXT == 16 && (TYT == 4 || TYT == 2), "16 Winograd tiles per workgroup tile: 4 x 4 or 2 x 8");
+  static constexpr bool DUST = DUST_, CONV = CONV_;
+  static_assert(TYT * TXT == 16 && (TYT == 4 || TYT == 2 || (CONV && !DUST && TYT == 8)), "16 Winograd tiles per workgroup tile: 4 x 4 or 2 x 8 (conv-only: or 8 x 2)");
   static constexpr int NT = 512, NTH = 256, NPOS = 36, KC = 16, N = 64;
   static constexpr int TH = 4 * TYT, TW = 4 * TXT, HH = TH + 2, HW = TW + 2, NHALO = HH * HW;
   static constexpr int HROW = 20;
@@ -25,13 +25,13 @@
   static constexpr int LDS_BYTES = LDS_FLOATS * 4;
   static_assert(LDS_BYTES <= 160 * 1024, "LDS");
   static constexpr int STEPS = 9;
-  static constexpr int WPAD = W36Cfg<1, TYT, TXT>::WPAD, WPAD2 = W36Cfg<1, TYT, TXT>::WPAD2;
+  static constexpr int WPAD = W36Cfg<1, 4, 4>::WPAD, WPAD2 = W36Cfg<1, 4, 4>::WPAD2;
   static_assert(WPAD >= 36, "a wave prefetches up to one chunk past its stream's end");
 };
 
-template <int TYT, int TXT, int RING, bool DUST>
+template <int TYT, int TXT, int RING, bool DUST, bool CONV = false>
 __device__ __forceinline__ void wblock36p_body(const WBlockArgs& a) {
-  using C = W36PCfg<TYT, TXT, DUST>;
+  using C = W36PCfg<TYT, TXT, DUST, CONV>;
   constexpr int TH = C::TH, TW = C::TW, HW = C::HW, HH = C::HH, HROW = C::HROW, HIT = C::HIT, NTH = C::NTH;
   constexpr int N = C::N, RH = C::RH, STEPS = C::STEPS, PX = C::PX;
   static_assert(STEPS % RING == 0 && RING >= 2, "ring slots must line up across chunks");
@@ -76,7 +76,8 @@
   auto slot_hyx = [&](int tl, int i) {
     const int e = tl + i * NTH;
     const int pix = (e * 13108) >> 16, c4 = e - pix * 5;
-    const int hy = HW == 18 ? (pix * 3641) >> 16 : (pix * 1928) >> 16;
+    const int hy = HW == 18 ? (pix * 3641) >> 16 : HW == 34 ? (pix * 1928) >> 16 : (pix * 6554) >> 16;
+    static_assert(HW == 18 || HW == 34 || HW == 10, "a division constant per halo width");
     const int hx = pix - hy * HW;
     const bool slot_ok = (hy < HH) & (c4 < 4);
     return slot_ok ? (hy << 16) | (c4 << 8) | hx : 0x7fff0000;
@@ -94,7 +95,7 @@
   [[maybe_unused]] int okoff64[C::HIT64];
   auto slot_hyx64 = [&](int tl, int i) {
     const int pix = tl + i * NTH;
-    const int hy = HW == 18 ? (pix * 3641) >> 16 : (pix * 1928) >> 16;
+    const int hy = HW == 18 ? (pix * 3641) >> 16 : HW == 34 ? (pix * 1928) >> 16 : (pix * 6554) >> 16;
     const int hx = pix - hy * HW;
     return (hy < HH && a.dust_in) ? (hy << 16) | hx : 0x7fff0000;
   };
@@ -539,7 +540,7 @@
         const int prow = i * RPI + rsub;
         if (prow < rows_valid) {
           f32x4 v = lds4[erd + i * PPI * (RH / 4)];
-          if (!a.conv_only) {
+          if (!CONV && !a.conv_only) {
             v.x = v.x > 0.f ? v.x : 0.f;
             v.y = v.y > 0.f ? v.y : 0.f;
             v.z = v.z > 0.f ? v.z : 0.f;
@@ -553,10 +554,10 @@
       }
     };
 
-    if (a.conv_only) {
+    if (CONV || a.conv_only) {
       store_out();
       FPC_LDS_BARRIER();
-    } else {
+    } else if constexpr (!CONV) {
       f32x4 acc2[8];
       const int pb = hs;
       [[maybe_unused]] float dpart[8];
@@ -743,6 +744,11 @@
 }
 
 template <int TYT, int TXT, int RING = 3>
+__global__ __launch_bounds__(512, 1) void wconv36p_kernel(const WBlockArgs a) {
+  wblock36p_body<TYT, TXT, RING, false, true>(a);
+}
+
+template <int TYT, int TXT, int RING = 3>
 __global__ __launch_bounds__(512, 1) void wblock36p_dust_kernel(const WBlockArgs a) {
   wblock36p_body<TYT, TXT, RING, true>(a);
 }
diff --git a/feature-point-cnn_amd/csrc/wblock_mfma.h b/feature-point-cnn_amd/csrc/wblock_mfma.h
--- a/feature-point-cnn_amd/csrc/wblock_mfma.h
+++ b/feature-point-cnn_amd/csrc/wblock_mfma.h
@@ -21,6 +21,7 @@
   int conv_only;
   const float* dust;
   int dust_in;
+  int frame_h;
 #ifdef FPC_DIAG
   unsigned long long* stamps;
 #endif
diff --git a/include/fpc.h b/include/fpc.h
--- a/include/fpc.h
+++ b/include/fpc.h
@@ -69,6 +69,7 @@
   FPC_PLAN_STEM_ROUND3 = 1 << 20,
   FPC_PLAN_CONV_ROUND1 = 1 << 21,
   FPC_PLAN_CONVT_PHASES = 1 << 19,
+  FPC_PLAN_TILES_ROUND5 = 1 << 22,
   FPC_PLAN_GUARD_ZONES = 1 << 15
 };
 
@@ -111,6 +112,8 @@
 int fpc_mark_weights_loaded(fpc_ctx* ctx);
 uint64_t fpc_plan_hash(const fpc_ctx* ctx);
 int fpc_pack_layout_revision(void);
+
+int fpc_tile_choice(int what, int H, int W, int frames, unsigned plan_flags);
 
 int fpc_check_guards(fpc_ctx* ctx, long long* bad_words);
 
```
